# opensensor/thingino-accel

Measured on AMD Instinct MI355X. Metric: images/sec yolov5s_int8 640x640 batch256, higher is better.
Workload: dtype int8

## Files before the change

thingino-accel_amd/csrc/hip/conv_i8.hip:

```cpp
#include "conv_i8_common.hpp"

#ifndef I8M_ABL
#define I8M_ABL 0
#endif
template <int BPX, int BN, int STAGES, int KS = 1, int NW = 4>
__global__ __launch_bounds__(NW * 64) void conv_i8_mfma(const mhip_conv_i8_t p, const long total_pix, const int k64,
                                                         const int8_t *__restrict__ zeros, const unsigned noc,
                                                         const unsigned nblk, const int lg_inc, const unsigned kw_magic,
                                                         const fastdiv_t dhw, const fastdiv_t dow, const int bufmode,
                                                         const unsigned in_bytes) {
    ANAT_BEGIN();
    const bool POW2 = lg_inc >= 0;
    const bool masked = p.kh * p.kw <= 32;
    constexpr int SLICE = (BPX + BN) * BK;
    constexpr int STAGE = KS * SLICE;
    constexpr int NWN = BN == 128 ? 2 : 1;
    constexpr int NWM = NW / NWN;
    constexpr int WPX = BPX / NWM / 16;
    constexpr int WOC = BN / NWN / 16;
    constexpr int XROWS = BPX / NW;
    constexpr int XI = XROWS / 16;
    constexpr int LW = (BN / 16 + NW - 1) / NW;
    constexpr int L = XI + LW;
    static_assert(XI >= 1 && XROWS % 16 == 0, "every wave fetches whole 16-row pieces of the pixel tile");
// ... 1034 lines not shown

static int launch_variant(const mhip_conv_i8_t *p, long total_pix, int k64, const variant_t &v) {
    if (v.persist < 0) return -1;
    if (v.rows) return conv_i8_launch_rows(p);
    if (v.r128) return launch_r128(p, total_pix, v.r128);
    if (v.patch) return conv_i8_launch_patch(p, k64, v.patch);
    const int bn = p->oc_pad % 128 == 0 ? 128 : (p->oc_pad % 64 == 0 ? 64 : 32);
    const bool b16 = v.persist && v.stages == 2 && bn16_ok(p);
    if (v.bpx == 256) {
        if (bn == 128) return launch_variant_t<256, 128>(p, total_pix, k64, v);
        if (bn == 64) return launch_variant_t<256, 64>(p, total_pix, k64, v);
        if (b16) return launch_variant_t<256, 16>(p, total_pix, k64, v);
        return launch_variant_t<256, 32>(p, total_pix, k64, v);
    }
    if (bn == 128) return launch_variant_t<128, 128>(p, total_pix, k64, v);
    if (bn == 64) return launch_variant_t<128, 64>(p, total_pix, k64, v);
    if (b16) return launch_variant_t<128, 16>(p, total_pix, k64, v);
    return launch_variant_t<128, 32>(p, total_pix, k64, v);
}

template <int BPX, int BN>
static int launch_pair_t(const mhip_conv_i8_t *a, const mhip_conv_i8_t *b, long total_pix, int k64, int lg, unsigned magic,
                         int wres) {
    if (a->nseg > 1) return -2;
    return launch_persist_t<BPX, BN, 2, true, false, true>(a, total_pix, k64, lg, magic, b, wres);
}
extern "C" int mhip_conv_i8_pair(const mhip_conv_i8_t *a, const mhip_conv_i8_t *b) {
    if (!a || !b || !tune().persist || tune().variant) return -2;
    if (a->in != b->in || a->in_stride != b->in_stride || a->frames != b->frames || a->in_h != b->in_h || a->in_w != b->in_w ||
        a->in_c != b->in_c || a->out_h != b->out_h || a->out_w != b->out_w || a->kh != b->kh || a->kw != b->kw ||
        a->stride_h != b->stride_h || a->stride_w != b->stride_w || a->pad_top != b->pad_top || a->pad_left != b->pad_left ||
        a->row_pad != b->row_pad || a->nseg != b->nseg || a->seg_up != b->seg_up || !a->lut || !b->lut || a->add || b->add ||
        a->out_nchw || b->out_nchw)
        return -2;
    for (int i = 0; i < a->nseg; i++)
        if (a->seg_in[i] != b->seg_in[i] || a->seg_c[i] != b->seg_c[i] || a->seg_stride[i] != b->seg_stride[i]) return -2;
    if ((a->in_c % 16) != 0 || mhip_conv_i8_small_c(a->in_c, a->kw, a->out_c) || mhip_conv_i8_small_c(b->in_c, b->kw, b->out_c))
        return -2;
    if (a->nseg > 1 && (!seg_valid(a) || !seg_valid(b))) return -2;
    if (!persist_eligible(a) || !persist_eligible(b)) return -2;
    const int bn = a->oc_pad % 128 == 0 ? 128 : (a->oc_pad % 64 == 0 ? 64 : 32);
    const int bnb = b->oc_pad % 128 == 0 ? 128 : (b->oc_pad % 64 == 0 ? 64 : 32);
    if (bn != bnb || !mhip_zero_page()) return -2;
    const long total_pix = (long)a->frames * a->out_h * a->out_w;
    const int k64 = (a->kh * a->row_pad + BK - 1) / BK * BK, nks = k64 / BK;
    if (total_pix <= 0 || total_pix > 0x7fffffffL) return -2;
    int lg = 0;
    while ((1 << lg) < a->in_c) lg++;
    const unsigned magic = ((65536u + (unsigned)a->kw - 1u) / (unsigned)a->kw);
    const variant_t dv = default_variant(a, nks);
    const int bpx = dv.bpx ? dv.bpx : 128, wres = dv.persist && dv.wres && (tune().wres & 2);
    const bool b16 = bn16_ok(a) && bn16_ok(b);
    if (bpx == 256) {
        if (bn == 128) return launch_pair_t<256, 128>(a, b, total_pix, k64, lg, magic, wres);
        if (bn == 64) return launch_pair_t<256, 64>(a, b, total_pix, k64, lg, magic, wres);
        if (b16) return launch_pair_t<256, 16>(a, b, total_pix, k64, lg, magic, wres);
        return launch_pair_t<256, 32>(a, b, total_pix, k64, lg, magic, wres);
    }
    if (bn == 128) return launch_pair_t<128, 128>(a, b, total_pix, k64, lg, magic, wres);
    if (bn == 64) return launch_pair_t<128, 64>(a, b, total_pix, k64, lg, magic, wres);
    if (b16) return launch_pair_t<128, 16>(a, b, total_pix, k64, lg, magic, wres);
    return launch_pair_t<128, 32>(a, b, total_pix, k64, lg, magic, wres);
}

extern "C" int mhip_conv_i8_seg_ok(const mhip_conv_i8_t *p) {
    return p && (p->in_c % 16) == 0 && !mhip_conv_i8_small_c(p->in_c, p->kw, p->out_c) && seg_valid(p) && persist_eligible(p);
}

extern "C" int mhip_conv_i8_variants(const mhip_conv_i8_t *p, int *codes, int max) {
    if (!p || (p->in_c % 16) != 0 || mhip_conv_i8_small_c(p->in_c, p->kw, p->out_c)) return 0;
    const int k64 = (p->kh * p->row_pad + BK - 1) / BK * BK, nks = k64 / BK;
    int n = 0;
    if (p->pre_w) {
        const int first = conv_i8_pre_tile_rows(p);
        for (int th : {first, 16, 8, 4})
            if (th && n < max && conv_i8_patch_ok(p, th, nullptr)) {
                const int code = th == 16 ? 10 : (th == 8 ? 9 : 11);
                bool seen = false;
                for (int i = 0; i < n; i++) seen |= codes[i] == code;
                if (!seen) codes[n++] = code;
            }
        return n;
    }
    if (p->nseg > 1) {
        const int bn = p->oc_pad % 128 == 0 ? 128 : (p->oc_pad % 64 == 0 ? 64 : 32);
        const variant_t dv = default_variant(p, nks);
        const int dflt = dv.persist && dv.wres ? (dv.bpx == 256 ? 15 : 14) : (dv.bpx == 256 ? 4 : 2);
        if (n < max) codes[n++] = dflt;
        if (n < max && dflt != 2) codes[n++] = 2;
        if (n < max && dflt != 4) codes[n++] = 4;
        if (n < max && dflt != 14 && LUTB + 2 * (size_t)128 * BK + (size_t)nks * bn * BK <= 80 * 1024) codes[n++] = 14;
        if (n < max && dflt != 15 && LUTB + 2 * (size_t)256 * BK + (size_t)nks * bn * BK <= 80 * 1024) codes[n++] = 15;
        return n;
    }
    const int dflt = variant_code(default_variant(p, nks));
    if (n < max) codes[n++] = dflt;
    for (int code = 1; code <= NVARIANTS; code++) {
        const variant_t v = variant_of(code);
        if (code == dflt) continue;
        if (v.patch && !conv_i8_patch_ok(p, v.patch, nullptr)) continue;
        if (v.persist && !persist_eligible(p)) continue;
        if (v.ks2 && ((nks & 1) || nks < 4 || p->oc_pad % 64 != 0)) continue;
        if (v.w8 && (p->oc_pad % 128 != 0 || nks < 3)) continue;
        if (v.persist < 0) continue;
        if (v.r128 && !r128_ok(p)) continue;
        if (v.rows && !conv_i8_rows_ok(p)) continue;
        if (v.wres) {
            const int bn = p->oc_pad % 128 == 0 ? 128 : (p->oc_pad % 64 == 0 ? 64 : 32);
            if (LUTB + 2 * (size_t)v.bpx * BK + (size_t)nks * bn * BK > 80 * 1024) continue;
        }
        if (!v.persist && v.stages == 3 && nks <= 2) continue;
        if (n < max) codes[n++] = code;
    }
    return n;
}

template <int BN>
static int launch_generic(const mhip_conv_i8_t *p, long total_pix, int k64) {
    dim3 grid((unsigned)((total_pix + BP - 1) / BP), (unsigned)(p->oc_pad / BN));
    hipLaunchKernelGGL((conv_i8_generic<BN>), grid, dim3(NTHREADS), 0, mhip_stream_native(), *p, total_pix, k64,
                       make_fastdiv((unsigned)(p->out_h * p->out_w)));
    return mhip_check(hipGetLastError(), "conv_i8_generic launch");
}

extern "C" int mhip_conv_i8(const mhip_conv_i8_t *p) {
    if (!p || !p->in || !p->out || !p->w) return -1;
    if (p->out_pix_stride < 0 || p->out_ch_off < 0 || (p->out_nchw && (p->out_pix_stride || p->out_ch_off)) ||
        (p->out_pix_stride && p->out_pix_stride < p->out_ch_off + p->out_c))
        return -1;
    if (p->frames <= 0 || p->in_h <= 0 || p->in_w <= 0 || p->in_c <= 0 || p->out_h <= 0 || p->out_w <= 0 ||
        p->out_c <= 0 || p->kh <= 0 || p->kw <= 0 || p->stride_h < 0 || p->stride_w < 0)
        return -1;
    int row_pad, oc_pad;
    mhip_conv_i8_pack_geom(p->in_c, p->kw, p->out_c, &row_pad, &oc_pad, nullptr);
    if (row_pad != p->row_pad || oc_pad != p->oc_pad) return -1;
    if (p->add && (!p->safe || p->out_nchw || ((p->out_c | p->out_pix_stride | p->out_ch_off) & 15) || (p->in_c % 16) != 0 ||
                   mhip_conv_i8_small_c(p->in_c, p->kw, p->out_c) || p->nseg > 1))
        return -1;
    const long total_pix = (long)p->frames * p->out_h * p->out_w;
    const int k64 = (p->kh * p->row_pad + BK - 1) / BK * BK;
    if (total_pix <= 0 || total_pix > 0x7fffffffL || (total_pix + BP - 1) / BP * (oc_pad / 32) > 0x7fffffffL) return -1;
    if (p->in_planar) {
        if (p->in_planar > 4 || p->in_c != 4 || p->in_w < 4 || p->stride_h < 1 || p->stride_w < 1 || p->add || p->nseg > 1 ||
            !mhip_conv_i8_small_c(p->in_c, p->kw, p->out_c))
            return -2;
        return conv_i8_try_smallc(p, k64);
    }
    if (mhip_conv_i8_small_c(p->in_c, p->kw, p->out_c)) {
        if (p->stride_h >= 1 && p->stride_w >= 1) {
            int rc = conv_i8_try_rgb(p, k64);
            if (rc == -2) rc = conv_i8_try_smallc(p, k64);
            if (rc != -2) return rc;
        }
        if (p->add || p->nseg > 1) return -1;
        if (oc_pad % 64 == 0) return launch_generic<64>(p, total_pix, k64);
        return launch_generic<32>(p, total_pix, k64);
    }
    if (p->pre_w) {
        if (!mhip_zero_page() || !mhip_conv_i8_pre_ok(p)) return -1;
        int th = conv_i8_pre_tile_rows(p);
        const int code = p->variant ? p->variant : tune().variant;
        if (code >= 9 && code <= 11) {
            const int want = code == 10 ? 16 : (code == 9 ? 8 : 4);
            if (conv_i8_patch_ok(p, want, nullptr)) th = want;
        } else if (tune().small_batch && conv_i8_patch_ok(p, 4, nullptr) &&
                   ((long)p->frames * p->out_h * p->out_w + 255) / 256 * ((p->oc_pad + 127) / 128) < 256) {
            th = 4;
        }
        return conv_i8_launch_patch(p, k64, th);
    }
    if ((p->in_c % 16) == 0) {
        if (!mhip_zero_page()) return -1;
        const int nks = k64 / BK;
        if (p->variant < 0 || p->variant > NVARIANTS) return -1;
        int code = p->variant;
        if (p->nseg > 1) {
            if (!seg_valid(p) || !persist_eligible(p)) return -1;
            if (!code && tune().variant) {
                int codes[NVARIANTS];
                const int n = mhip_conv_i8_variants(p, codes, NVARIANTS);
                for (int i = 0; i < n; i++)
                    if (codes[i] == tune().variant) code = codes[i];
            }
            variant_t v = variant_of(code == 4 || code == 14 || code == 15 ? code : 2);
            if (!code) {
                const variant_t dv = default_variant(p, nks);
                v.bpx = dv.bpx ? dv.bpx : 128;
                v.wres = dv.persist && dv.wres;
            }
            return launch_variant(p, total_pix, k64, v);
        }
        if (!code && tune().variant) {
            int codes[NVARIANTS];
            const int n = mhip_conv_i8_variants(p, codes, NVARIANTS);
            for (int i = 0; i < n; i++)
                if (codes[i] == tune().variant) code = codes[i];
        }
        return launch_variant(p, total_pix, k64, code ? variant_of(code) : default_variant(p, nks));
    }
    if (oc_pad % 64 == 0) return launch_generic<64>(p, total_pix, k64);
    return launch_generic<32>(p, total_pix, k64);
}
```

thingino-accel_amd/csrc/hip/conv_i8_common.hpp:

```cpp
#pragma once
#include <hip/hip_runtime.h>
#include <stdint.h>
#include <stdlib.h>
#include <string.h>
#include <type_traits>

#include "../mhip.h"

extern "C" hipStream_t mhip_stream_native(void);
extern "C" int mhip_check(hipError_t e, const char *what);
extern "C" const void *mhip_zero_page(void);

typedef int v4i __attribute__((ext_vector_type(4)));
typedef int v2i __attribute__((ext_vector_type(2)));

#ifdef ANATOMY
struct anat_rec_t {
    unsigned key, wg, hwid, xcc;
    unsigned long long t[4];
};
static __device__ anat_rec_t *g_anat_buf;
static __device__ unsigned g_anat_cap;
#define ANAT_SETTER(NAME)                                                                                                    \
    extern "C" int NAME(void *buf, unsigned cap) {                                                                          \
// ... 318 lines not shown
                __builtin_memcpy(d, &v, 16);
            } else {
                const int rem = ncols - c * 16;
                int o = 0;
                if (rem & 8) { __builtin_memcpy(d, s, 8); o = 8; }
                if (rem & 4) { __builtin_memcpy(d + o, s + o, 4); o += 4; }
                if (rem & 2) { __builtin_memcpy(d + o, s + o, 2); o += 2; }
                if (rem & 1) d[o] = s[o];
            }
        }
    } else {
        for (int id = tid; id < BPX * BN; id += (int)blockDim.x) {
            const int c = id / BPX, row = id - c * BPX;
            const long off = rowoff[row];
            if (off < 0 || c >= ncols) continue;
            p.out[off + (size_t)(oc0 + c) * hw] = tile[row * ROW + c];
        }
    }
}

template <int BPX, int BN, int WPX, int WOC, bool LUT0 = false>
__device__ __forceinline__ void epilogue(const mhip_conv_i8_t &p, v4i (&acc)[WOC][WPX], int8_t *tile, const uint8_t *slut,
                                         const long *rowoff, int oc0, int pxw, int ocw, int hw) {
    const bool direct = !p.out_nchw && ((p.out_c | p.out_pix_stride | p.out_ch_off) & 15) == 0;
#define EPI(L, S, D) epilogue_t<BPX, BN, WPX, WOC, L, S, D, LUT0>(p, acc, tile, slut, rowoff, oc0, pxw, ocw, hw)
    if (direct) {
        if (p.lut) { if (p.safe) EPI(true, true, true); else EPI(true, false, true); }
        else { if (p.safe) EPI(false, true, true); else EPI(false, false, true); }
    } else {
        if (p.lut) { if (p.safe) EPI(true, true, false); else EPI(true, false, false); }
        else { if (p.safe) EPI(false, true, false); else EPI(false, false, false); }
    }
#undef EPI
}

template <int WPX, int WOC>
__device__ __forceinline__ void init_acc(const mhip_conv_i8_t &p, v4i (&acc)[WOC][WPX], int ocbase) {
    const int lane = threadIdx.x & 63;
#pragma unroll
    for (int s = 0; s < WOC; s++) {
        const v4i b = p.bias ? *(const v4i *)(p.bias + ocbase + s * 16 + (lane >> 4) * 4) : (v4i){0, 0, 0, 0};
#pragma unroll
        for (int t = 0; t < WPX; t++) acc[s][t] = b;
    }
}


struct tune_t {
    int init;
    int persist;
    int persist_stages;
    int persist_maxk;
    int persist_slots;
    int stages;
    int bpx;
    int variant;
    int bufmode;
    int small_batch;
    int rgb_direct;
    int wres;
    int few_wgs;
    int rows;
    int patch_ring;
    int patch_lds_kb;
};
const tune_t &conv_i8_tune_state();

extern "C" int mhip_conv_i8_small_c(int in_c, int kw, int out_c);

static inline long in_extent_bytes(const mhip_conv_i8_t *p) {
    return (long)(p->frames - 1) * (long)p->in_stride + (long)p->in_h * p->in_w * p->in_c;
}
static inline long persist_out_bytes(const mhip_conv_i8_t *p) {
    const long pstride = p->out_pix_stride ? p->out_pix_stride : p->out_c;
    return (long)(p->frames - 1) * (long)p->out_stride + (long)p->out_h * p->out_w * pstride;
}
static inline bool conv_i8_direct_rows(const mhip_conv_i8_t *p) {
    return !p->out_nchw && ((p->out_c | p->out_pix_stride | p->out_ch_off) & 15) == 0;
}

bool conv_i8_patch_ok(const mhip_conv_i8_t *p, int th, int *ring);
int conv_i8_launch_patch(const mhip_conv_i8_t *p, int k64, int th);
int conv_i8_pre_tile_rows(const mhip_conv_i8_t *p);
bool conv_i8_rows_ok(const mhip_conv_i8_t *p);
int conv_i8_launch_rows(const mhip_conv_i8_t *p);
int conv_i8_try_rgb(const mhip_conv_i8_t *p, int k64);
int conv_i8_try_smallc(const mhip_conv_i8_t *p, int k64);
```

thingino-accel_amd/csrc/hip/conv_i8_patch.hip:

```cpp
#include "conv_i8_common.hpp"
#include <stdio.h>

#ifdef PATCH_STAMPS
__device__ unsigned long long patch_stamp_sums[8];
extern "C" int mhip_patch_stamps(unsigned long long *out, int reset) {
    if (out && hipMemcpyFromSymbol(out, HIP_SYMBOL(patch_stamp_sums), sizeof(patch_stamp_sums)) != hipSuccess) return -1;
    if (reset) {
        unsigned long long z[8] = {0};
        if (hipMemcpyToSymbol(HIP_SYMBOL(patch_stamp_sums), z, sizeof(z)) != hipSuccess) return -1;
    }
    return 0;
}
#define STAMP(t)                                                                          \
    do {                                                                                  \
        __builtin_amdgcn_sched_barrier(0);                                                \
        asm volatile("s_memtime %0\n\ts_waitcnt lgkmcnt(0)" : "=s"(t)::"memory");        \
        __builtin_amdgcn_sched_barrier(0);                                                \
    } while (0)
#else
#define STAMP(t) do { } while (0)
#endif
#define PT_TW 16
#define PT_NIMAX 10

template <int LO, int HI>
__device__ __forceinline__ void wait_vmcnt_tree(int n) {
    if constexpr (LO == HI) {
        wait_vmcnt<LO>();
    } else {
        constexpr int MID = (LO + HI + 1) / 2;
        if (n >= MID) wait_vmcnt_tree<MID, HI>(n);
        else wait_vmcnt_tree<LO, MID - 1>(n);
    }
}
template <int HI>
__device__ __forceinline__ void wait_vmcnt_upto(int n) {
    wait_vmcnt_tree<0, HI>(n > HI ? HI : n);
}
__device__ __forceinline__ void barrier_lds() {
    asm volatile("s_waitcnt lgkmcnt(0)\n\ts_barrier" ::: "memory");
}

template <int TH, int BN, bool HAS_LUT, bool PRE = false>
__global__ __launch_bounds__(NTHREADS) void conv_i8_patch(const mhip_conv_i8_t p, const int k64, const int tiles_x,
                                                          const int tiles_y, const unsigned ntiles_all, const int PH,
                                                          const int PW, const int PWP, const int PWH, const int nblk,
                                                          const int8_t *__restrict__ zeros, const fastdiv_t dtx,
                                                          const fastdiv_t dty, const fastdiv_t dpwp, const unsigned out_bytes,
                                                          const int ring, const int xmap, const unsigned in_bytes) {
    ANAT_BEGIN();
    constexpr int WPX = TH / 4;
    constexpr int WOC = BN / 16;
    constexpr int NST = WPX;
    extern __shared__ __attribute__((aligned(16))) int8_t dynlds[];
    uint8_t *slut = (uint8_t *)dynlds;
    lds_base_must_be_zero(dynlds);
    const int nks = k64 / BK;
    constexpr int LB = LUTB + (PRE ? 512 : 0);
    int *dutab = (int *)(dynlds + LB);
    int8_t *wl = dynlds + LB + ((nks * 16 + 255) & ~255);
    const int patch_bytes = nblk * 1024;
    int8_t *w1l = wl + nks * BN * BK;
    int8_t *patch0 = w1l + (PRE ? p.in_c * BK : 0);
    int8_t *tpatch = patch0 + ring * patch_bytes;

    const int tid = threadIdx.x, lane = tid & 63;
    const int wv = __builtin_amdgcn_readfirstlane(tid >> 6);
    const int oc0 = blockIdx.y * BN;
    const int C = p.in_c, lgc = 31 - __builtin_clz((unsigned)C), cpp = C >> 4, lgcpp = lgc - 4;
    const int s = p.stride_w;
    const unsigned M = C >= 128 ? 6u : (C >= 64 ? 2u : 0u);

    v4i bias[WOC];
#pragma unroll
    for (int q = 0; q < WOC; q++) bias[q] = p.bias ? *(const v4i *)(p.bias + oc0 + q * 16 + (lane >> 4) * 4) : (v4i){0, 0, 0, 0};
    constexpr int W1MAX = 4;
    v4i pbias[PRE ? W1MAX : 1];
    if (PRE) {
#pragma unroll
        for (int q = 0; q < W1MAX; q++) pbias[q] = q < (C >> 4) ? *(const v4i *)(p.pre_bias + q * 16 + (lane >> 4) * 4) : (v4i){0, 0, 0, 0};
    }
    if (HAS_LUT) {
        if (p.lut2) { if (tid < 128) ((uint32_t *)slut)[tid] = ((const uint32_t *)p.lut2)[tid]; }
        else if (tid < 64) ((uint32_t *)slut)[tid] = ((const uint32_t *)p.lut)[tid];
    }
    if (PRE && tid >= 128) ((uint32_t *)slut)[tid] = ((const uint32_t *)p.pre_lut2)[tid - 128];
    const int rowbytes = p.kw * C, kbytes = p.kh * rowbytes;
    for (int i = tid; i < nks * 4; i += NTHREADS) {
        const int kb = i * 16;
        int du = 0;
        if (kb < kbytes) {
            const int ky = kb / rowbytes, rem = kb - ky * rowbytes, kx = rem >> lgc, cc = (rem & (C - 1)) >> 4;
            const int dp = ky * PWP + (s == 2 ? (kx >> 1) + (kx & 1) * PWH : kx);
            du = dp * cpp + cc;
        }
        dutab[i] = du;
    }
    __syncthreads();
    {
        const int schunk = (lane & 3) ^ (((lane >> 4) & 1) << 1);
        for (int i = wv; i < nks * (BN / 16); i += 4) {
            const int ks = i / (BN / 16), g = i - ks * (BN / 16);
            glds16(p.w + (size_t)(oc0 + g * 16 + (lane >> 2)) * k64 + ks * BK + schunk * 16, wl + (ks * BN + g * 16) * BK);
        }
        if (PRE)
            for (int g = wv; g < C / 16; g += 4) glds16(p.pre_w + (size_t)(g * 16 + (lane >> 2)) * BK + schunk * 16, w1l + g * 16 * BK);
    }
    int uoff[PT_NIMAX], upos[PT_NIMAX];
#pragma unroll
    for (int n = 0; n < PT_NIMAX; n++) {
        uoff[n] = 0;
        upos[n] = -1;
        if (n * 4 + wv < nblk) {
            const unsigned phys = (unsigned)((n * 4 + wv) * 64 + lane);
            const unsigned U = phys ^ ((phys >> 3) & M);
            const unsigned pp = U >> lgcpp, cc = U & (unsigned)(cpp - 1);
            const unsigned py = fdiv(pp, dpwp), col = pp - py * (unsigned)PWP;
            const int px = s == 2 ? ((int)col < PWH ? 2 * (int)col : 2 * ((int)col - PWH) + 1) : (int)col;
            if ((int)py < PH && px < PW) {
                uoff[n] = ((int)py * p.in_w + px) * C + (int)cc * 16;
                upos[n] = ((int)py << 16) | px;
            }
        }
    }
    const int npw = nblk > wv ? (nblk - wv + 3) >> 2 : 0;
    const unsigned xcd = blockIdx.x & 7u;
    const unsigned xstart = xmap ? (unsigned)(((unsigned long long)ntiles_all * xcd) >> 3) : 0u;
    const unsigned xend = xmap ? (unsigned)(((unsigned long long)ntiles_all * (xcd + 1u)) >> 3) : 0u;
    const unsigned ntiles = xmap ? (xend - xstart) * 8u + xcd : ntiles_all;
    auto tile_xy = [&](unsigned t, int &tx, int &ty, unsigned &f) {
        const unsigned j = xmap ? xstart + (t >> 3) : t, q = fdiv(j, dtx);
        tx = (int)(j - q * (unsigned)tiles_x);
        f = fdiv(q, dty);
        ty = (int)(q - f * (unsigned)tiles_y);
    };
    const __amdgpu_buffer_rsrc_t xrs = __builtin_amdgcn_make_buffer_rsrc((void *)p.in, 0, (int)in_bytes, 0x00020000);
    auto issue_patch = [&](unsigned t, int8_t *dst) {
#ifdef PATCH_ABL
        return;
#endif
        int tx, ty;
        unsigned f;
        tile_xy(t, tx, ty, f);
        const int iy0 = ty * TH * s - p.pad_top, ix0 = tx * PT_TW * s - p.pad_left;
        if (in_bytes != 0u && iy0 >= 0 && ix0 >= 0 && iy0 + PH <= p.in_h && ix0 + PW <= p.in_w) {
            const int sbase = (int)(f * (unsigned)p.in_stride) + (iy0 * p.in_w + ix0) * C;
#pragma unroll
            for (int n = 0; n < PT_NIMAX; n++)
                if (n * 4 + wv < nblk) blds16(xrs, uoff[n], sbase, dst + (n * 4 + wv) * 1024);
            return;
        }
        const int8_t *base = p.in + (size_t)f * p.in_stride + ((long)iy0 * p.in_w + ix0) * C;
#pragma unroll
        for (int n = 0; n < PT_NIMAX; n++)
            if (n * 4 + wv < nblk) {
                const int py = upos[n] >> 16, px = upos[n] & 0xffff;
                const bool ok = upos[n] >= 0 && (unsigned)(iy0 + py) < (unsigned)p.in_h && (unsigned)(ix0 + px) < (unsigned)p.in_w;
                glds16(ok ? base + uoff[n] : zeros, dst + (n * 4 + wv) * 1024);
            }
    };

    const __amdgpu_buffer_rsrc_t orsrc = __builtin_amdgcn_make_buffer_rsrc(p.out, 0, (int)out_bytes, 0x00020000);
    const bool has_add = p.add != nullptr;
    constexpr int RROW = WOC == 4 ? 1024 : 512;
    constexpr int NRI = WOC == 4 ? WPX : 2 * WPX;
    int8_t *rstage = patch0 + (ring + (PRE ? 1 : 0)) * patch_bytes + wv * (WPX * RROW);
    const int NR = has_add ? NRI : 0;
    const int frow = lane & 15, fchunk = lane >> 4;
    const int chan = (lane >> 4) * (4 * WOC);
    const int pstride = p.out_pix_stride ? p.out_pix_stride : p.out_c;
    const int lo = p.relu ? 0 : -128;
    const uint8_t *lut128 = slut + 128;
    int ubase[WPX];
#pragma unroll
    for (int u = 0; u < WPX; u++) ubase[u] = ((wv * WPX + u) * s * PWP + frow) * cpp;

    const unsigned G = gridDim.x;
    const int D = ring - 1;
    unsigned t = blockIdx.x;
    int yg0 = 0, yg1 = 0, yg2 = 0;
    {
        int issued = 0;
        for (int d = 0; d < D; d++)
            if (t + (unsigned)d * G < ntiles) {
                issue_patch(t + (unsigned)d * G, patch0 + d * patch_bytes);
                issued++;
            }
        yg0 = issued > 1 ? (issued - 1) * npw : 0;
        yg1 = issued > 2 ? (issued - 2) * npw : 0;
        yg2 = 0;
    }
#ifdef PATCH_STAMPS
    unsigned long long st0 = 0, st1 = 0, st2 = 0, st3 = 0, st4 = 0, sum_wait = 0, sum_issue = 0, sum_k = 0, sum_epi = 0, sum_tiles = 0;
#endif
    int cur = 0;
    int pn_last = 0;
    bool first = true;
    ANAT_NOW(1);
    for (; t < ntiles; t += G) {
        STAMP(st0);
        int tx, ty;
        unsigned f;
        tile_xy(t, tx, ty, f);
        int voffs[WPX];
        uint32_t xw[WPX][WOC];
#pragma unroll
        for (int u = 0; u < WPX; u++) {
            const int oy = ty * TH + wv * WPX + u, ox = tx * PT_TW + frow;
            const unsigned off = f * (unsigned)p.out_stride + (unsigned)(oy * p.out_w + ox) * (unsigned)pstride +
                                 (unsigned)(p.out_ch_off + oc0 + chan);
            const bool ok = oy < p.out_h && ox < p.out_w && oc0 + chan < p.out_c;
            voffs[u] = ok ? (int)off : -1;
#pragma unroll
            for (int q = 0; q < WOC; q++) xw[u][q] = 0;
        }
        if (has_add) {
#pragma unroll
            for (int u = 0; u < WPX; u++) {
                const int8_t *src = voffs[u] >= 0 ? p.add + (unsigned)voffs[u] : zeros;
                if (WOC == 4) {
                    glds16(src, rstage + u * RROW);
                } else {
                    __builtin_amdgcn_global_load_lds((const __attribute__((address_space(1))) void *)src,
                                                     (__attribute__((address_space(3))) void *)(rstage + u * RROW), 4, 0, 0);
                    __builtin_amdgcn_global_load_lds((const __attribute__((address_space(1))) void *)(src + 4),
                                                     (__attribute__((address_space(3))) void *)(rstage + u * RROW + 256), 4, 0, 0);
                }
            }
        }
        if (D > 0) {
            wait_vmcnt_upto<63>(yg0 + NR);
            barrier_lds();
            STAMP(st1);
            const unsigned tn = t + (unsigned)D * G;
            int pn = 0;
            if (tn < ntiles) {
                int slot = cur + D;
                slot = slot >= ring ? slot - ring : slot;
                issue_patch(tn, patch0 + slot * patch_bytes);
                pn = npw;
            }
            const int after = NR + pn + NST;
            yg0 = yg1 + after;
            yg1 = yg2 + after;
            yg2 = NST;
            if (D == 1) yg0 = NST;
            if (D == 2) yg1 = NST;
            pn_last = pn;
        } else {
            if (!first) barrier_lds();
            issue_patch(t, patch0);
            wait_vmcnt<0>();
            barrier_lds();
        }
        first = false;
        STAMP(st2);
        const int8_t *patch = patch0 + cur * patch_bytes;
        if (PRE) {
            const int WOC1 = C >> 4;
            const int P = PH * PWP, nsub = (P + 15) >> 4;
            const int iy0 = ty * TH * s - p.pad_top, ix0 = tx * PT_TW * s - p.pad_left;
            for (int sub = wv; sub < nsub; sub += 4) {
                int pp = sub * 16 + frow;
                const bool live = pp < P;
                pp = live ? pp : P - 1;
                const unsigned Ur = (unsigned)(pp * cpp + (fchunk & (cpp - 1)));
                const v4i xb1 = *(const v4i *)(patch + ((Ur ^ ((Ur >> 3) & M)) << 4));
                const unsigned py = fdiv((unsigned)pp, dpwp), px = (unsigned)pp - py * (unsigned)PWP;
                const bool inimg = live && (int)py < PH && (int)px < PW && (unsigned)(iy0 + (int)py) < (unsigned)p.in_h &&
                                   (unsigned)(ix0 + (int)px) < (unsigned)p.in_w;
                uint32_t pk1[W1MAX];
                if (WOC1 == 4) {
                    int a1[16];
#pragma unroll
                    for (int q = 0; q < 4; q++) {
                        const v4i wa = *(const v4i *)(w1l + lds_off(q * 16 + frow, fchunk));
                        const v4i r = __builtin_amdgcn_mfma_i32_16x16x64_i8(wa, xb1, pbias[PRE ? q : 0], 0, 0, 0);
#pragma unroll
                        for (int e = 0; e < 4; e++) a1[q * 4 + e] = r[e];
                    }
                    uint32_t pk4[4];
                    requant_pack_pre<16>(a1, p.pre_cs, pk4);
#pragma unroll
                    for (int e = 0; e < 4; e++) pk1[e] = inimg ? pk4[e] : 0u;
                    const unsigned Uw = (unsigned)(pp * cpp + (lane >> 4));
                    if (live) *(v4i *)(tpatch + ((Uw ^ ((Uw >> 3) & M)) << 4)) = (v4i){(int)pk1[0], (int)pk1[1], (int)pk1[2], (int)pk1[3]};
                } else {
                    int a1[8];
#pragma unroll
                    for (int q = 0; q < 2; q++) {
                        const v4i wa = *(const v4i *)(w1l + lds_off(q * 16 + frow, fchunk));
                        const v4i r = __builtin_amdgcn_mfma_i32_16x16x64_i8(wa, xb1, pbias[PRE ? q : 0], 0, 0, 0);
#pragma unroll
                        for (int e = 0; e < 4; e++) a1[q * 4 + e] = r[e];
                    }
                    uint32_t pk2[2];
                    requant_pack_pre<8>(a1, p.pre_cs, pk2);
                    const int g4 = lane >> 4;
                    const unsigned Uw = (unsigned)(pp * cpp + (g4 >> 1));
                    if (live)
                        *(uint2 *)(tpatch + ((Uw ^ ((Uw >> 3) & M)) << 4) + (g4 & 1) * 8) = make_uint2(inimg ? pk2[0] : 0u, inimg ? pk2[1] : 0u);
                }
            }
            barrier_lds();
            patch = tpatch;
        }
        v4i acc[WOC][WPX];
        v4i xa[WPX], wa[WOC], xb[WPX], wb[WOC];
        auto load_frags = [&](int ks, int du, v4i (&xf)[WPX], v4i (&wf)[WOC]) {
#pragma unroll
            for (int u = 0; u < WPX; u++) {
                const unsigned U = (unsigned)(ubase[u] + du);
                xf[u] = *(const v4i *)(patch + ((U ^ ((U >> 3) & M)) << 4));
            }
            const int8_t *ws = wl + ks * BN * BK;
#pragma unroll
            for (int q = 0; q < WOC; q++) wf[q] = *(const v4i *)(ws + lds_off(q * 16 + frow, fchunk));
        };
        auto mfma_step = [&](const v4i (&xf)[WPX], const v4i (&wf)[WOC]) {
#pragma unroll
            for (int q = 0; q < WOC; q++)
#pragma unroll
                for (int u = 0; u < WPX; u++) acc[q][u] = __builtin_amdgcn_mfma_i32_16x16x64_i8(wf[q], xf[u], acc[q][u], 0, 0, 0);
        };
        const int last = nks - 1;
        auto clampk = [&](int k) { return k < last ? k : last; };
        load_frags(0, dutab[fchunk], xa, wa);
        load_frags(clampk(1), dutab[clampk(1) * 4 + fchunk], xb, wb);
        int du_n = dutab[clampk(2) * 4 + fchunk];
#pragma unroll
        for (int q = 0; q < WOC; q++)
#pragma unroll
            for (int u = 0; u < WPX; u++) acc[q][u] = __builtin_amdgcn_mfma_i32_16x16x64_i8(wa[q], xa[u], bias[q], 0, 0, 0);
        int ks = 1;
        for (; ks + 1 < nks; ks += 2) {
            load_frags(ks + 1, du_n, xa, wa);
            du_n = dutab[clampk(ks + 2) * 4 + fchunk];
            __builtin_amdgcn_sched_barrier(0);
            mfma_step(xb, wb);
            __builtin_amdgcn_sched_barrier(0);
            load_frags(clampk(ks + 2), du_n, xb, wb);
            du_n = dutab[clampk(ks + 3) * 4 + fchunk];
            __builtin_amdgcn_sched_barrier(0);
            mfma_step(xa, wa);
            __builtin_amdgcn_sched_barrier(0);
        }
        if (ks < nks) mfma_step(xb, wb);
        STAMP(st3);
        if (D > 0) cur = cur + 1 == ring ? 0 : cur + 1;
        if (has_add) {
            if (D > 0) wait_vmcnt_upto<15>(pn_last);
#pragma unroll
            for (int u = 0; u < WPX; u++) {
                if (WOC == 4) {
                    const v4i r = *(const v4i *)(rstage + u * RROW + lane * 16);
                    xw[u][0] = (uint32_t)r[0]; xw[u][1] = (uint32_t)r[1]; xw[u][WOC > 2 ? 2 : 0] = (uint32_t)r[2]; xw[u][WOC > 3 ? 3 : 0] = (uint32_t)r[3];
                } else {
                    xw[u][0] = *(const uint32_t *)(rstage + u * RROW + lane * 4);
                    xw[u][WOC > 1 ? 1 : 0] = *(const uint32_t *)(rstage + u * RROW + 256 + lane * 4);
                }
            }
        }
#pragma unroll
        for (int u = 0; u < WPX; u++) {
            uint32_t pk[WOC];
            int a[WOC * 4];
#pragma unroll
            for (int q = 0; q < WOC; q++)
#pragma unroll
                for (int r = 0; r < 4; r++) a[q * 4 + r] = acc[q][u][r];
            const bool fast = HAS_LUT && p.lut2 != nullptr;
            if (has_add) {
                const add_args_t ga = {p.add_s_conv, p.add_s_other, p.add_inv};
                if (fast) requant_pack<WOC * 4, HAS_LUT, true, true, true, true>(a, p.cs, lo, lut128, pk, xw[u], &ga);
                else requant_pack<WOC * 4, HAS_LUT, true, true, true>(a, p.cs, lo, lut128, pk, xw[u], &ga);
            } else {
                if (fast) requant_pack<WOC * 4, HAS_LUT, true, true, false, true>(a, p.cs, lo, lut128, pk);
                else requant_pack<WOC * 4, HAS_LUT, true, true>(a, p.cs, lo, lut128, pk);
            }
            const int voff = voffs[u];
            if (WOC == 4)
                __builtin_amdgcn_raw_buffer_store_b128((v4i){(int)pk[0], (int)pk[1], (int)pk[2], (int)pk[3]}, orsrc, voff, 0, 0);
            else if (WOC == 2)
                __builtin_amdgcn_raw_buffer_store_b64((v2i){(int)pk[0], (int)pk[WOC > 1 ? 1 : 0]}, orsrc, voff, 0, 0);
        }
#ifdef PATCH_STAMPS
        STAMP(st4);
        if (D == 0) st1 = st2;
        sum_wait += st1 - st0; sum_issue += st2 - st1; sum_k += st3 - st2; sum_epi += st4 - st3; sum_tiles += 1;
#endif
    }
    ANAT_NOW(2);
    ANAT_END(p);
#ifdef PATCH_STAMPS
    if (lane == 0) {
        atomicAdd(&patch_stamp_sums[0], sum_wait); atomicAdd(&patch_stamp_sums[1], sum_issue); atomicAdd(&patch_stamp_sums[2], sum_k);
        atomicAdd(&patch_stamp_sums[3], sum_epi); atomicAdd(&patch_stamp_sums[4], sum_tiles);
    }
#endif
}

ANAT_SETTER(mhip_anatomy_set_patch)
struct patch_geom_t {
    int bn, tiles_x, tiles_y, PH, PW, PWP, PWH, nblk, nks, ring;
    size_t lds;
};
static inline const tune_t &tune() { return conv_i8_tune_state(); }
static size_t patch_lds_budget(int bn) {
    const int kb = tune().patch_lds_kb;
    if (kb >= 16 && kb <= 160 && kb != 80) return (size_t)kb * 1024;
    return (size_t)(bn == 32 ? 53 : 80) * 1024;
}
static bool patch_geom(const mhip_conv_i8_t *p, int th, patch_geom_t *g) {
    const bool direct = conv_i8_direct_rows(p);
    const int C = p->in_c, s = p->stride_w;
    static const bool no_c16 = getenv("MARS_HIP_PATCH_NO_C16") != nullptr;
    if (!direct || !p->safe || (C != 16 && C != 32 && C != 64 && C != 128) || (C == 16 && (no_c16 || p->pre_w)) || (s != 1 && s != 2) || p->stride_h != s ||
        p->kh > 7 || p->kw > 7 || p->kh * p->kw < 2 || p->row_pad != p->kw * C || persist_out_bytes(p) > 0x7fffffffL)
        return false;
    const int k64 = (p->kh * p->row_pad + BK - 1) / BK * BK;
    g->nks = k64 / BK;
    g->bn = p->oc_pad % 64 == 0 ? 64 : 32;
    g->tiles_x = (p->out_w + PT_TW - 1) / PT_TW;
    g->tiles_y = (p->out_h + th - 1) / th;
    if ((double)p->out_h * p->out_w < (C == 128 ? 0.80 : 0.85) * (double)g->tiles_x * PT_TW * g->tiles_y * th) return false;
    g->PH = (th - 1) * s + p->kh;
    g->PW = (PT_TW - 1) * s + p->kw;
    g->PWH = s == 2 ? (g->PW + 1) / 2 : 0;
    g->PWP = s == 2 ? 2 * g->PWH : g->PW;
    const long units = (long)g->PH * g->PWP * (C / 16);
    g->nblk = (int)((units + 63) / 64);
    if (g->nblk > 4 * PT_NIMAX) return false;
    const bool pre = p->pre_w != nullptr;
    if (pre && (s != 1 || (C != 32 && C != 64) || !p->pre_bias || !p->pre_lut2 || !p->lut2)) return false;
    const size_t pb = (size_t)g->nblk * 1024;
    const size_t radd = p->add ? (size_t)4 * (th / 4) * (g->bn == 64 ? 1024 : 512) : 0;
    const size_t fixed = LUTB + (pre ? 512 + (size_t)C * BK + pb : 0) + (((size_t)g->nks * 16 + 255) & ~(size_t)255) +
                         (size_t)g->nks * g->bn * BK + radd;
    const size_t budget = patch_lds_budget(g->bn);
    if (fixed + pb > budget) return false;
    const int fit = (int)((budget - fixed) / pb);
    const int cap = tune().patch_ring > 0 ? (tune().patch_ring > 4 ? 4 : tune().patch_ring) : 2;
    int ring = fit < cap ? fit : cap;
    g->ring = ring;
    g->lds = fixed + (size_t)ring * pb;
    if ((long)g->tiles_x * g->tiles_y * p->frames > 0x7fffffffL) return false;
    return true;
}

template <int TH, int BN, bool HAS_LUT, bool PRE = false>
static int launch_patch_t(const mhip_conv_i8_t *p, int k64, const patch_geom_t &g) {
    auto kern = conv_i8_patch<TH, BN, HAS_LUT, PRE>;
    static int cus = 0;
    static size_t slots_lds[8];
    static int slots_n[8], nslots = 0;
    if (!cus) {
        int dev = 0;
        hipDeviceProp_t prop;
        if (hipFuncSetAttribute((const void *)kern, hipFuncAttributeMaxDynamicSharedMemorySize, 160 * 1024) != hipSuccess ||
            hipGetDevice(&dev) != hipSuccess || hipGetDeviceProperties(&prop, dev) != hipSuccess)
            return mhip_check(hipErrorUnknown, "conv_i8_patch occupancy query");
        cus = prop.multiProcessorCount;
    }
    int slots = 0;
    for (int i = 0; i < nslots; i++)
        if (slots_lds[i] == g.lds) slots = slots_n[i];
    if (!slots) {
        int occ = 0;
        if (hipOccupancyMaxActiveBlocksPerMultiprocessor(&occ, kern, NTHREADS, g.lds) != hipSuccess)
            return mhip_check(hipErrorUnknown, "conv_i8_patch occupancy query");
        slots = (occ > 0 ? occ : 1) * cus;
        if (nslots < 8) { slots_lds[nslots] = g.lds; slots_n[nslots++] = slots; }
    }
    const unsigned ntiles = (unsigned)((long)g.tiles_x * g.tiles_y * p->frames);
    const unsigned noc = (unsigned)(p->oc_pad / BN);
    unsigned gx = (unsigned)(tune().persist_slots > 0 ? tune().persist_slots : slots) / noc;
    if (gx < 1) gx = 1;
    if (gx > ntiles) gx = ntiles;
    const int xmap = gx >= 8 && ntiles < 0x0fffffffu;
    if (xmap) gx &= ~7u;
    {
        static const char *dbg = getenv("MARS_HIP_PATCH_DEBUG");
        static size_t last_lds = 0;
        static int last_ring = 0;
        if (dbg && (last_lds != g.lds || last_ring != g.ring)) {
            fprintf(stderr, "Mars: conv_i8_patch<%d,%d> ring %d, patch %d KB, LDS %zu B, %d workgroups per CU, grid %u x %u\n", TH, BN, g.ring,
                    g.nblk, g.lds, slots / cus, gx, noc);
            last_lds = g.lds;
            last_ring = g.ring;
        }
    }
    hipLaunchKernelGGL(kern, dim3(gx, noc), dim3(NTHREADS), g.lds, mhip_stream_native(), *p, k64,
                       g.tiles_x, g.tiles_y, ntiles, g.PH, g.PW, g.PWP, g.PWH, g.nblk, (const int8_t *)mhip_zero_page(),
                       make_fastdiv((unsigned)g.tiles_x), make_fastdiv((unsigned)g.tiles_y), make_fastdiv((unsigned)g.PWP),
                       (unsigned)persist_out_bytes(p), g.ring, xmap,
                       in_extent_bytes(p) <= 0x7fffffffL ? (unsigned)in_extent_bytes(p) : 0u);
    return mhip_check(hipGetLastError(), "conv_i8_patch launch");
}

bool conv_i8_patch_ok(const mhip_conv_i8_t *p, int th, int *ring) {
    patch_geom_t g;
    if (!patch_geom(p, th, &g)) return false;
    if (ring) *ring = g.ring;
    return true;
}

int conv_i8_launch_patch(const mhip_conv_i8_t *p, int k64, int th) {
    patch_geom_t g;
    if (!patch_geom(p, th, &g)) return -1;
#define PATCH(T, B)                                                                       \
    (p->pre_w ? launch_patch_t<T, B, true, true>(p, k64, g)                               \
              : (p->lut ? launch_patch_t<T, B, true>(p, k64, g) : launch_patch_t<T, B, false>(p, k64, g)))
    if (th == 16) return g.bn == 64 ? PATCH(16, 64) : PATCH(16, 32);
    if (th == 8) return g.bn == 64 ? PATCH(8, 64) : PATCH(8, 32);
    return g.bn == 64 ? PATCH(4, 64) : PATCH(4, 32);
#undef PATCH
}

int conv_i8_pre_tile_rows(const mhip_conv_i8_t *p) {
    patch_geom_t g;
    for (int th : {16, 8, 4})
        if (patch_geom(p, th, &g) && (th == 4 || g.ring >= 2)) return th;
    return 0;
}
extern "C" int mhip_conv_i8_pre_ok(const mhip_conv_i8_t *p) {
    if (!p || !p->pre_w || p->nseg > 1 || p->out_nchw) return 0;
    return conv_i8_pre_tile_rows(p) != 0;
}
```

thingino-accel_amd/csrc/host/mars_internal.h:

```cpp
#ifndef MARS_INTERNAL_H
#define MARS_INTERNAL_H

#include <stddef.h>
#include <stdint.h>

#include "../mhip.h"
#include "mars_hip.h"
#include "mars_runtime.h"

enum {
    OP_CONV_I8 = 0,
    OP_CONV_F32,
    OP_RELU_BYTES,
    OP_LUT_I8,
    OP_BINARY_I8,
    OP_SIGMOID_F32,
    OP_BINARY_F32,
    OP_RELU_F32,
    OP_BN,
    OP_MAXPOOL,
    OP_CONCAT_SLICE,
    OP_UPSAMPLE,
    OP_UPSAMPLE_Q, OP_MAXPOOL_Q,
    OP_CONCAT_Q,
    OP_CONV_F32_VHEAD,
    OP_FAIL,
};

#define NO_OFF ((size_t)-1)
#define MARS_MAX_IO 4
#define MARS_MAX_MODEL_TUNE 16

typedef struct {
    size_t bytes;
    size_t extent;
    size_t stride;
    uint8_t *dev;
    int is_weight;
    int needed;
    int io_in, io_out;
    uint8_t *host;
    uint8_t *dense_dev;
    int pix_c, pix_stride;
    int rec_c, rec_hw;
    int nhwc_c, nhwc_hw;
    size_t zero_from;
    int partial;
    int nhwc_pitch;
    int tail_read;
} mtensor_t;

typedef struct {
    int kind, layer, err;
    int t_in[4], n_in, t_out;
    int in_h, in_w, in_c, out_h, out_w, out_c, kh, kw, sh, sw, pt, pl;
    int nchw, relu, is_mul, is_f32, leaky, safe;
    size_t in_byte_off, out_byte_off;
    int k_limit;
    int vc_n, vc_t[3], vc_run, vc_shift;
    int rows_only;
    int out_nchw;
    int silu_f32;
    int f32_exact;
    int variant;
    int add_t; float add_s_conv, add_s_other, add_inv;
    int nseg, seg_t[4], seg_c[4], seg_up;
    int chain_n, chain_out[3];
    int pair_next;
    int row_pad, oc_pad, c_pad;
    int ch_off, scale_h, scale_w, bn_n;
    int out_pix_stride, out_ch_off;
    int store_c;
    float cs, f0, f1, f2;
    size_t n;
    size_t w_off, b_off, lut_off, s_off;
    int pre;
    size_t pre_w_off, pre_b_off, pre_lut2_off;
    float pre_cs;
    size_t w2_off;
    int w2_rows;
    int w2_planes;
    size_t w3_off;
    int w3_stem;
    int in_rec, out_rec;
    size_t lut2_off;
    size_t w_blob_off[2];
    double macs, bytes;
    int prof_kind;
    float last_ms;
    void *ev0, *ev1;
    int prof_rec;
    void *ev_start;
} mars_op_t;

typedef struct {
    int fusion;
    unsigned no_fuse_lut : 1, no_nhwc_internal : 1, no_vconcat_q : 1, no_pair_f32 : 1, no_rec : 1, no_zero_tail : 1, no_vconcat_f32 : 1,
        no_rowpad : 1;
    size_t rec_limit;
    size_t vconcat_limit;
    size_t bottleneck_limit;
} plan_switches_t;

typedef struct mars_model_ext {
    mars_model_t pub;
    plan_switches_t sw;
    int batch, profiling, deferred;
    int plan_err;
    int no_vconcat;
    int no_download;
    int no_bottleneck;
    int rec_frames;
    int rec_skipped;
    size_t rec_max_frames;
    mtensor_t *mt;
    mars_op_t *ops;
    int n_ops, cap_ops;
    uint8_t *arena_host;
    size_t arena_size, arena_cap;
    uint8_t *arena_dev;
    size_t blob_mirror_bytes;
    uint8_t *act_dev;
    size_t act_bytes;
    uint8_t *scratch_dev;
    size_t scratch_per_frame;
    int scratch_t, scratch_cpad, scratch_f0, scratch_n;
    void *det_dev;
    int *det_counts_dev;
    float *det_lut_dev;
    int det_cap;
    float det_lut_scale[4];
    int det_lut_n;
    int det_lut_mono[4];
    float *heads_lut_dev;
    float heads_lut_scale[4];
    int heads_lut_n;
    float *dfl_lut_dev;
    float dfl_lut_scale[4][2];
    int dfl_lut_n;
    void *ev_graph_done, *ev_tail_done;
    int tail_pending;
    int frame0, run_frames;
    void *ev_fork, *ev_join[3];
    void *ev_chunk[2][8];
    void *graph_exec;
    unsigned graph_gen;
    int ran_plain;
    void *pipe;
    struct { char key[28]; int value, saved; } tune[MARS_MAX_MODEL_TUNE];
    int n_tune, tune_depth;
    int plan_f32_mode;
    unsigned char *layer_noop;
    void *roi_dev;
    int roi_cap_slots, roi_cap_frames;
    int roi_slots;
    struct mars_model_ext *roi_from;
    void *cls_dev;
    size_t cls_bytes, cls_sums_off, cls_top_off;
    int cls_frames, cls_c, cls_top_k;
    void *ev_label_done;
    int label_pending;
    void *label_dev;
    int label_cap, label_frames;
    void *match_dev;
    size_t match_bytes, match_top_off, match_row_off;
    int match_frames, match_top_k;
    void *ident_dev;
    int ident_cap, ident_frames;
    void *track_dev;
    int track_cap, track_frames;
    void *seg_dev;
    size_t seg_bytes, seg_rec_off, seg_word_off;
    int seg_frames, seg_max, seg_ph, seg_pw;
    void *ev_seg[2];
    void *pose_dev;
    size_t pose_bytes, pose_rec_off, pose_kpt_off;
    int pose_frames, pose_max, pose_k;
    float pose_lut_scale[4];
    int pose_lut_n;
    void *ev_pose[2];
    struct mars_model_ext *live_next;
} mars_model_ext_t;


#define MARS_INTERNAL __attribute__((visibility("hidden")))
#define ALIGN_UP(x, a) (((x) + (size_t)(a) - 1) & ~((size_t)(a) - 1))
#define NO_TENSOR 0xFFFFFFFFu
#define MAX_DIM_PRODUCT ((size_t)1 << 40)
#define ARENA_MAX ((size_t)1 << 40)
#define MAX_CHANNELS 65536
MARS_INTERNAL int mars_verbose(void);
#define VLOG(...) do { if (mars_verbose()) fprintf(stderr, "Mars: " __VA_ARGS__); } while (0)
MARS_INTERNAL void drop_graph(mars_model_ext_t *m);
MARS_INTERNAL mars_model_ext_t *mars_live_models(void);
MARS_INTERNAL void plan_switches_read(plan_switches_t *sw, int at_load);
MARS_INTERNAL mars_error_t build_plan(mars_model_ext_t *m);
MARS_INTERNAL mars_error_t upload_params(mars_model_ext_t *m);
MARS_INTERNAL mars_error_t alloc_batch(mars_model_ext_t *m, int n);
MARS_INTERNAL size_t elem_size(uint32_t dtype);
MARS_INTERNAL size_t shape_numel(const mars_tensor_t *d);
MARS_INTERNAL size_t reference_buffer_size(const mars_model_ext_t *m);
MARS_INTERNAL size_t arena_reserve(mars_model_ext_t *m, size_t bytes);
MARS_INTERNAL void blob_read(const mars_model_ext_t *m, size_t off, size_t n, void *dst);
MARS_INTERNAL int op_reads(const mars_op_t *o, int t);
MARS_INTERNAL int op_writes(const mars_op_t *o, int t);
MARS_INTERNAL size_t planned_stride(const mtensor_t *t);
MARS_INTERNAL void conv_i8_geometry(const mars_op_t *op, int frames, mhip_conv_i8_t *p);
MARS_INTERNAL int conv_i8_pre_fits(const mars_op_t *op, int frames, size_t in_stride, size_t out_stride);
MARS_INTERNAL void plan_layer(mars_model_ext_t *m, int li);
MARS_INTERNAL void fold_silu(mars_model_ext_t *m, int f32);
MARS_INTERNAL void fuse_lut(mars_model_ext_t *m);
MARS_INTERNAL void nhwc_internal(mars_model_ext_t *m);
MARS_INTERNAL void fold_add(mars_model_ext_t *m, int f32);
MARS_INTERNAL void virtual_concat(mars_model_ext_t *m);
MARS_INTERNAL void elide_concat(mars_model_ext_t *m);
MARS_INTERNAL void trim_concat(mars_model_ext_t *m);
MARS_INTERNAL void fuse_pool_chains(mars_model_ext_t *m);
MARS_INTERNAL void pair_convs(mars_model_ext_t *m);
MARS_INTERNAL void fuse_bottleneck(mars_model_ext_t *m);
MARS_INTERNAL void pad_output_rows(mars_model_ext_t *m);
MARS_INTERNAL void virtual_concat_q(mars_model_ext_t *m);
MARS_INTERNAL void f32_policy(mars_model_ext_t *m);
MARS_INTERNAL void zero_tail_f32(mars_model_ext_t *m);
MARS_INTERNAL void pair_convs_f32(mars_model_ext_t *m);
MARS_INTERNAL void rec_pairs(mars_model_ext_t *m);
MARS_INTERNAL void virtual_concat_f32(mars_model_ext_t *m);
MARS_INTERNAL void plan_check(mars_model_ext_t *m);
MARS_INTERNAL void conv_i8_params(const mars_model_ext_t *m, const mars_op_t *op, mhip_conv_i8_t *p);
MARS_INTERNAL int mars_preproc_prepare(int w, int h, int tw, int th);
MARS_INTERNAL int mars_preproc_prepare_nv12(int w, int h, int tw, int th, int frames);

MARS_INTERNAL void mars_roi_release(mars_model_ext_t *m);

MARS_INTERNAL void mars_cls_release(mars_model_ext_t *m);

MARS_INTERNAL void mars_match_release(mars_model_ext_t *m);

MARS_INTERNAL void mars_track_release(mars_model_ext_t *m);

MARS_INTERNAL void mars_seg_release(mars_model_ext_t *m);

MARS_INTERNAL void mars_pose_release(mars_model_ext_t *m);

MARS_INTERNAL int mars_tensor_chw(const mars_tensor_t *d, int *c, int *h, int *w);
MARS_INTERNAL int mars_locate_i8(const mars_model_ext_t *m, int T, int ch, int hh, int ww, int any_writer, int *buf, int *off, int *pix_step, int *ch_step);
MARS_INTERNAL mars_error_t mars_own_det_buffers(mars_model_ext_t *m);
MARS_INTERNAL mars_error_t mars_tail_on_aux(mars_model_ext_t *m, int (*launch)(struct mars_model_ext *, const void *, void *, int *), const void *cfg);

mars_error_t mars_detect_prepare(mars_model_ext_t *m, const int *output_indices, int n_outputs);
int mars_detect_launch(mars_model_ext_t *m, const int *output_indices, int n_outputs, float nms_thresh, void *dets_dev,
                       int *counts_dev);

typedef struct {
    int n, ti[4], stride[4], nc[4], h[4], w[4], pix_step[4], ch_step[4];
    float anchors[4][3][2];
    float conf, nms;
    int map, px, py;
    float rx, ry;
    int internal;
} mars_heads_cfg_t;
MARS_INTERNAL int mars_find_heads(const mars_model_ext_t *m, int *tensor_ids, int *strides, int *num_classes, int cap);
MARS_INTERNAL mars_error_t mars_heads_resolve(mars_model_ext_t *m, const mars_yolo_heads_t *h, mars_heads_cfg_t *c);
MARS_INTERNAL mars_error_t mars_heads_prepare(mars_model_ext_t *m, const mars_heads_cfg_t *c);
MARS_INTERNAL int mars_heads_launch(mars_model_ext_t *m, const mars_heads_cfg_t *c, void *dets_dev, int *counts_dev);

typedef struct {
    int n, reg_max, stride[4], nc[4], h[4], w[4];
    int box_t[4], cls_t[4], box_buf[4], cls_buf[4], box_off[4], cls_off[4];
    int box_pix_step[4], box_ch_step[4], cls_pix_step[4], cls_ch_step[4];
    float box_scale[4], cls_scale[4];
    float conf, nms;
    int map, px, py;
    float rx, ry;
    int internal;
    int *cand_pred, *kept_pred;
    void *premap;
} mars_dfl_cfg_t;
MARS_INTERNAL int mars_find_dfl_heads(const mars_model_ext_t *m, int *box_ids, int *cls_ids, int *strides, int *num_classes, int *reg_max, int cap);
MARS_INTERNAL mars_error_t mars_dfl_resolve(mars_model_ext_t *m, const mars_yolo_dfl_heads_t *h, mars_dfl_cfg_t *c);
MARS_INTERNAL mars_error_t mars_dfl_prepare(mars_model_ext_t *m, const mars_dfl_cfg_t *c);
MARS_INTERNAL int mars_dfl_launch(mars_model_ext_t *m, const mars_dfl_cfg_t *c, void *dets_dev, int *counts_dev);

int32_t mars_trunc_x86(float x);
void mars_pack_conv_i8(const int8_t *w, size_t avail, int nchw, int out_c, int in_c, int kh, int kw,
                       int c_pad, int row_pad, int oc_pad, int8_t *dst);

#endif
```

thingino-accel_amd/csrc/host/mars_model.c:

```c
#include <math.h>
#include <stdio.h>
#include <stdlib.h>
#include <string.h>
#include <sys/types.h>
#include <time.h>

#include "mars_internal.h"
#include "nna.h"


int mars_verbose(void) {
    static int v = -1;
    if (v < 0) v = getenv("MARS_VERBOSE") ? 1 : 0;
    return v;
}

void plan_switches_read(plan_switches_t *sw, int at_load) {
    const char *e;
    if (at_load) sw->fusion = (e = getenv("MARS_HIP_FUSION")) ? atoi(e) : 1;
    sw->no_fuse_lut = getenv("MARS_HIP_NO_FUSE_LUT") != NULL;
    sw->no_nhwc_internal = getenv("MARS_HIP_NO_NHWC_INTERNAL") != NULL;
    sw->no_vconcat_q = getenv("MARS_HIP_NO_VCONCAT_Q") != NULL;
    sw->no_pair_f32 = getenv("MARS_HIP_NO_PAIR_F32") != NULL;
    sw->no_rec = getenv("MARS_HIP_NO_REC") != NULL;
    sw->no_zero_tail = getenv("MARS_HIP_NO_ZERO_TAIL") != NULL;
    sw->no_vconcat_f32 = getenv("MARS_HIP_NO_VCONCAT_F32") != NULL;
    sw->no_rowpad = getenv("MARS_HIP_NO_ROWPAD") != NULL;
    sw->rec_limit = (e = getenv("MARS_HIP_REC_LIMIT")) ? (size_t)strtoull(e, NULL, 0) : (size_t)0xfffffff0u;
    sw->vconcat_limit = (e = getenv("MARS_HIP_VCONCAT_LIMIT")) ? (size_t)strtoull(e, NULL, 0) : (size_t)0x7fffffffu;
    sw->bottleneck_limit = (e = getenv("MARS_HIP_BOTTLENECK_LIMIT")) ? (size_t)strtoull(e, NULL, 0) : 0;
}

void drop_graph(mars_model_ext_t *m) {
    if (m->graph_exec) {
        mhip_sync();
        mhip_graph_destroy(m->graph_exec);
    }
    m->graph_exec = NULL;
    m->ran_plain = 0;
}

static const char *const k_err[] = {
    "OK", "Invalid magic number", "Version mismatch", "Memory allocation failed",
    "Invalid file format", "NNA initialization failed", "Layer execution failed",
    "Invalid tensor", "Invalid layer",
};

const char *mars_get_error_string(mars_error_t err) {
    int i = -(int)err;
    if (i >= 0 && i < (int)(sizeof(k_err) / sizeof(k_err[0]))) return k_err[i];
    return "Unknown error";
}

static void free_device_state(mars_model_ext_t *m) {
    drop_graph(m);
    if (m->act_dev) mhip_free(m->act_dev);
    if (m->scratch_dev) mhip_free(m->scratch_dev);
    m->act_dev = m->scratch_dev = NULL;
    for (uint32_t i = 0; m->mt && i < m->pub.header.num_tensors; i++) {
        if (m->mt[i].host) mhip_host_free(m->mt[i].host);
        m->mt[i].host = NULL;
        if (m->mt[i].dense_dev) mhip_free(m->mt[i].dense_dev);
        m->mt[i].dense_dev = NULL;
        if (!m->mt[i].is_weight) m->mt[i].dev = NULL;
    }
    if (m->det_dev) mhip_free(m->det_dev);
    if (m->det_counts_dev) mhip_free(m->det_counts_dev);
    m->det_dev = NULL;
    m->det_counts_dev = NULL;
    m->det_cap = 0;
    m->tail_pending = 0;
    mars_roi_release(m);
    mars_cls_release(m);
    mars_track_release(m);
    mars_seg_release(m);
    mars_pose_release(m);
}

static void free_ops(mars_model_ext_t *m) {
    drop_graph(m);
    for (int i = 0; i < m->n_ops; i++) {
        if (m->ops[i].ev0) mhip_event_destroy(m->ops[i].ev0);
        if (m->ops[i].ev1) mhip_event_destroy(m->ops[i].ev1);
    }
    free(m->ops);
    m->ops = NULL;
    m->n_ops = m->cap_ops = 0;
}

static mars_model_ext_t *g_live_models = NULL;
mars_model_ext_t *mars_live_models(void) { return g_live_models; }

void mars_free(mars_model_t *model) {
    if (!model) return;
    mars_model_ext_t *m = (mars_model_ext_t *)model;
    for (mars_model_ext_t **pp = &g_live_models; *pp; pp = &(*pp)->live_next)
        if (*pp == m) { *pp = m->live_next; break; }
    for (mars_model_ext_t *x = g_live_models; x; x = x->live_next)
        if (x->roi_from == m) x->roi_from = NULL;
    if (m->pipe) mars_hip_pipe_close(model);
    if (mhip_ready()) mhip_sync();
    free_device_state(m);
    free_ops(m);
    if (m->arena_dev) mhip_free(m->arena_dev);
    if (m->det_lut_dev) mhip_free(m->det_lut_dev);
    if (m->heads_lut_dev) mhip_free(m->heads_lut_dev);
    if (m->dfl_lut_dev) mhip_free(m->dfl_lut_dev);
    if (m->ev_graph_done) mhip_event_destroy(m->ev_graph_done);
    if (m->ev_tail_done) mhip_event_destroy(m->ev_tail_done);
    if (m->ev_label_done) mhip_event_destroy(m->ev_label_done);
    if (m->ev_fork) mhip_event_destroy(m->ev_fork);
    for (int k = 0; k < 3; k++)
        if (m->ev_join[k]) mhip_event_destroy(m->ev_join[k]);
    for (int k = 0; k < 2; k++)
        for (int c = 0; c < 8; c++)
            if (m->ev_chunk[k][c]) mhip_event_destroy(m->ev_chunk[k][c]);
    free(m->arena_host);
    free(m->layer_noop);
    free(m->mt);
    free(m->pub.weights);
    free(m->pub.layers);
    free(m->pub.tensors);
    free(m);
}

mars_error_t build_plan(mars_model_ext_t *m) {
    const uint32_t nt = m->pub.header.num_tensors, nl = m->pub.header.num_layers;
    plan_switches_read(&m->sw, 0);
    free_ops(m);
    m->arena_size = 0;
    if (m->arena_host) memset(m->arena_host, 0, m->arena_cap);
    m->scratch_per_frame = 0;
    m->plan_err = MARS_OK;
    m->plan_f32_mode = mhip_conv_f32_mode(-1);
    m->blob_mirror_bytes = m->pub.weights_size;
    for (uint32_t i = 0; i < nt; i++) {
        m->mt[i].extent = m->mt[i].bytes;
        m->mt[i].pix_c = m->mt[i].pix_stride = 0;
        m->mt[i].needed = (m->mt[i].io_in || m->mt[i].io_out) ? 1 : 0;
    }
    for (uint32_t i = 0; i < nl && m->plan_err == MARS_OK; i++) {
        const int n0 = m->n_ops;
        plan_layer(m, (int)i);
        m->layer_noop[i] = m->n_ops == n0;
    }
    if (m->plan_err != MARS_OK) return (mars_error_t)m->plan_err;
    if (m->sw.fusion >= 1) {
        fold_silu(m, 0);
        fuse_lut(m);
        fold_silu(m, 1);
        nhwc_internal(m);
        fold_add(m, 0);
        fold_add(m, 1);
        if (!m->no_vconcat) virtual_concat(m);
        elide_concat(m);
        trim_concat(m);
        fuse_pool_chains(m);
        pair_convs(m);
        if (m->sw.fusion >= 2 && !m->no_bottleneck) fuse_bottleneck(m);
        pad_output_rows(m);
        virtual_concat_q(m);
    } else {
        nhwc_internal(m);
    }
    f32_policy(m);
    zero_tail_f32(m);
    if (m->sw.fusion >= 1) pair_convs_f32(m);
    rec_pairs(m);
    virtual_concat_f32(m);
    if (m->plan_err == MARS_OK) plan_check(m);
    return (mars_error_t)m->plan_err;
}

mars_error_t upload_params(mars_model_ext_t *m) {
    size_t mirror_off = arena_reserve(m, m->blob_mirror_bytes + 64);
    if (mirror_off == NO_OFF) return MARS_ERR_ALLOC_FAILED;
    if (!m->deferred) blob_read(m, 0, m->blob_mirror_bytes, m->arena_host + mirror_off);
    if (m->arena_dev) mhip_free(m->arena_dev);
    m->arena_dev = (uint8_t *)mhip_malloc(m->arena_size);
    if (!m->arena_dev) return MARS_ERR_ALLOC_FAILED;
    if (mhip_h2d_async(m->arena_dev, m->arena_host, m->arena_size) || mhip_sync()) return MARS_ERR_NNA_INIT_FAILED;
    for (uint32_t i = 0; i < m->pub.header.num_tensors; i++) {
        if (!m->mt[i].is_weight) continue;
        m->mt[i].dev = m->arena_dev + mirror_off + (size_t)m->pub.tensors[i].desc.data_offset;
        m->mt[i].stride = 0;
        m->pub.tensors[i].paddr = m->mt[i].dev;
    }
    m->pub.ddr_paddr = m->arena_dev;
    m->pub.ddr_size = m->arena_size;
    return MARS_OK;
}

mars_error_t alloc_batch(mars_model_ext_t *m, int n) {
    const uint32_t nt = m->pub.header.num_tensors;
    if (m->pipe) mars_hip_pipe_close(&m->pub);
    if (mhip_sync()) return MARS_ERR_LAYER_FAILED;
    plan_switches_read(&m->sw, 0);
    const size_t vlim = m->sw.vconcat_limit, blim = m->sw.bottleneck_limit;
    const int rec_replan = (size_t)n > m->rec_max_frames || (m->rec_skipped && n < m->rec_frames);
    m->rec_frames = n;
    if (m->no_vconcat || m->no_bottleneck || rec_replan) {
        m->no_vconcat = m->no_bottleneck = 0;
        mars_error_t e = build_plan(m);
        if (e == MARS_OK) e = upload_params(m);
        if (e != MARS_OK) return e;
    }
    if (!m->no_vconcat)
        for (int i = 0; i < m->n_ops; i++) {
            const mars_op_t *op = &m->ops[i];
            if (op->kind != OP_CONV_I8 || op->nseg < 2 || op->t_out < 0) continue;
            if (planned_stride(&m->mt[op->t_out]) * (size_t)n > vlim) {
                m->no_vconcat = 1;
                mars_error_t e = build_plan(m);
                if (e == MARS_OK) e = upload_params(m);
                if (e != MARS_OK) return e;
                break;
            }
        }
    if (m->sw.fusion >= 2 && !m->no_bottleneck)
        for (int i = 0; i < m->n_ops; i++) {
            const mars_op_t *op = &m->ops[i];
            if (op->kind != OP_CONV_I8 || !op->pre || op->t_out < 0) continue;
            const size_t in_stride = op->t_in[0] >= 0 ? planned_stride(&m->mt[op->t_in[0]]) : 0;
            if (!conv_i8_pre_fits(op, n, in_stride, planned_stride(&m->mt[op->t_out])) || (blim && (size_t)n > blim)) {
                m->no_bottleneck = 1;
                mars_error_t e = build_plan(m);
                if (e == MARS_OK) e = upload_params(m);
                if (e != MARS_OK) return e;
                break;
            }
        }
    free_device_state(m);
    size_t per_frame = 0;
    for (uint32_t i = 0; i < nt; i++) {
        mtensor_t *t = &m->mt[i];
        if (t->is_weight || !t->needed) continue;
        t->stride = planned_stride(t);
        per_frame += t->stride;
    }
    m->act_bytes = per_frame * (size_t)n;
    m->act_dev = (uint8_t *)mhip_malloc(m->act_bytes + 512);
    if (!m->act_dev) return MARS_ERR_ALLOC_FAILED;
    if (mhip_memset_async(m->act_dev, 0, m->act_bytes + 256)) return MARS_ERR_ALLOC_FAILED;
    size_t off = 256;
    for (uint32_t i = 0; i < nt; i++) {
        mtensor_t *t = &m->mt[i];
        mars_runtime_tensor_t *rt = &m->pub.tensors[i];
        if (t->is_weight) continue;
        rt->vaddr = NULL; rt->paddr = NULL; rt->alloc_size = 0;
        if (!t->needed) continue;
        t->dev = m->act_dev + off;
        off += t->stride * (size_t)n;
        rt->paddr = t->dev;
        rt->alloc_size = t->stride * (size_t)n;
        if (t->io_in || t->io_out) {
            const size_t hb = t->bytes * (size_t)n, ref = reference_buffer_size(m);
            size_t cap = hb > ref ? hb : ref;
            if (ref > ((size_t)8 << 20)) cap = hb;
            t->host = (uint8_t *)mhip_host_alloc(cap ? cap : 64);
            if (!t->host) return MARS_ERR_ALLOC_FAILED;
            memset(t->host, 0, cap);
            rt->vaddr = t->host;
            rt->alloc_size = n == 1 && cap >= ref ? ref : hb;
        }
        if (t->pix_stride) {
            t->dense_dev = (uint8_t *)mhip_malloc(t->bytes * (size_t)n);
            if (!t->dense_dev) return MARS_ERR_ALLOC_FAILED;
        }
    }
    if (m->scratch_per_frame) {
        m->scratch_dev = (uint8_t *)mhip_malloc(ALIGN_UP(m->scratch_per_frame, 256) * (size_t)n + 256);
        if (!m->scratch_dev) return MARS_ERR_ALLOC_FAILED;
    }
    m->batch = n;
    m->frame0 = 0;
    m->run_frames = n;
    return mhip_sync() ? MARS_ERR_ALLOC_FAILED : MARS_OK;
}

static mars_error_t load_host(const void *data, size_t size, unsigned flags, mars_model_ext_t **out_m) {
    if (!data || !out_m || size < sizeof(mars_header_t)) return MARS_ERR_INVALID_FILE;
    const uint8_t *p = (const uint8_t *)data;
    mars_header_t h;
    memcpy(&h, p, sizeof(h));
    if (h.magic != MARS_MAGIC) {
        VLOG("Invalid magic 0x%08x (expected 0x%08x)\n", h.magic, MARS_MAGIC);
        return MARS_ERR_INVALID_MAGIC;
    }
    if (h.version_major != MARS_VERSION_MAJOR) return MARS_ERR_VERSION_MISMATCH;
    if (h.num_tensors > 65536 || h.num_layers > 65536 || h.num_inputs > 4 || h.num_outputs > 4) return MARS_ERR_INVALID_FILE;
    const size_t tables = sizeof(h) + (size_t)h.num_tensors * sizeof(mars_tensor_t) + (size_t)h.num_layers * sizeof(mars_layer_t);
    if (tables > size) return MARS_ERR_INVALID_FILE;
    const int deferred = (flags & MARS_HIP_LOAD_DEFER_WEIGHTS) != 0;
    if (!deferred && h.weights_size > 0 && (h.weights_offset > size || h.weights_size > size - h.weights_offset))
        return MARS_ERR_INVALID_FILE;
    if (h.weights_size > ((uint64_t)1 << 36)) return MARS_ERR_INVALID_FILE;

    mars_model_ext_t *m = (mars_model_ext_t *)calloc(1, sizeof(*m));
    if (!m) return MARS_ERR_ALLOC_FAILED;
    m->pub.header = h;
    plan_switches_read(&m->sw, 1);
    m->deferred = deferred;
    m->pub.tensors = (mars_runtime_tensor_t *)calloc(h.num_tensors ? h.num_tensors : 1, sizeof(mars_runtime_tensor_t));
    m->pub.layers = (mars_runtime_layer_t *)calloc(h.num_layers ? h.num_layers : 1, sizeof(mars_runtime_layer_t));
    m->mt = (mtensor_t *)calloc(h.num_tensors ? h.num_tensors : 1, sizeof(mtensor_t));
    m->layer_noop = (unsigned char *)calloc(h.num_layers ? h.num_layers : 1, 1);
    if (!m->pub.tensors || !m->pub.layers || !m->mt || !m->layer_noop) { mars_free(&m->pub); return MARS_ERR_ALLOC_FAILED; }
    const uint8_t *q = p + sizeof(h);
    for (uint32_t i = 0; i < h.num_tensors; i++, q += sizeof(mars_tensor_t)) memcpy(&m->pub.tensors[i].desc, q, sizeof(mars_tensor_t));
    for (uint32_t i = 0; i < h.num_layers; i++, q += sizeof(mars_layer_t)) memcpy(&m->pub.layers[i].desc, q, sizeof(mars_layer_t));

    m->pub.weights_size = (size_t)h.weights_size;
    if (h.weights_size) {
        m->pub.weights = calloc(1, (size_t)h.weights_size);
        if (!m->pub.weights) { mars_free(&m->pub); return MARS_ERR_ALLOC_FAILED; }
        if (!deferred) memcpy(m->pub.weights, p + h.weights_offset, (size_t)h.weights_size);
    }
    m->pub.ddr_base = m->pub.weights;
    for (uint32_t i = 0; i < h.num_tensors; i++) {
        mars_runtime_tensor_t *rt = &m->pub.tensors[i];
        if (rt->desc.ndims > MARS_MAX_DIMS) { mars_free(&m->pub); return MARS_ERR_INVALID_FILE; }
        m->mt[i].bytes = shape_numel(&rt->desc) * elem_size(rt->desc.dtype);
        if (rt->desc.data_size > 0) {
            if (rt->desc.data_offset > h.weights_size) { mars_free(&m->pub); return MARS_ERR_INVALID_FILE; }
            m->mt[i].is_weight = 1;
            rt->vaddr = (uint8_t *)m->pub.weights + rt->desc.data_offset;
            rt->alloc_size = (size_t)rt->desc.data_size;
        }
    }
    for (uint32_t i = 0; i < h.num_inputs; i++) {
        uint32_t id = h.input_tensor_ids[i];
        if (id < h.num_tensors && !m->mt[id].is_weight) m->mt[id].io_in = (int)i + 1;
    }
    for (uint32_t i = 0; i < h.num_outputs; i++) {
        uint32_t id = h.output_tensor_ids[i];
        if (id < h.num_tensors && !m->mt[id].is_weight) m->mt[id].io_out = (int)i + 1;
    }

    mars_error_t err = build_plan(m);
    if (err != MARS_OK) { mars_free(&m->pub); return err; }
    VLOG("%u layers -> %d launches, parameter arena %zu bytes\n", h.num_layers, m->n_ops, m->arena_size);
    *out_m = m;
    return MARS_OK;
}

mars_error_t mars_hip_load_memory_ex(const void *data, size_t size, unsigned flags, mars_model_t **out_model) {
    if (!out_model) return MARS_ERR_INVALID_FILE;
    mars_model_ext_t *m = NULL;
    mars_error_t err = load_host(data, size, flags, &m);
    if (err != MARS_OK) return err;
    if (!nna_is_ready() || !mhip_ready()) {
        fprintf(stderr, "Mars: no initialised MI355X device (call nna_init first); refusing to load\n");
        mars_free(&m->pub);
        return MARS_ERR_NNA_INIT_FAILED;
    }
    err = upload_params(m);
    if (err == MARS_OK) err = alloc_batch(m, 1);
    if (err != MARS_OK) { mars_free(&m->pub); return err; }
    m->live_next = g_live_models;
    g_live_models = m;
    *out_model = &m->pub;
    return MARS_OK;
}

static int describe_op_full(const mars_op_t *o, char *line, size_t cap, int k) {
#define ADD(...) k += snprintf(line + k, cap - (size_t)k, __VA_ARGS__)
    ADD(" | err %d in %dx%dx%d out %dx%dx%d k %dx%d s %dx%d p %d,%d", o->err, o->in_h, o->in_w, o->in_c, o->out_h, o->out_w, o->out_c, o->kh, o->kw, o->sh, o->sw, o->pt, o->pl);
    ADD(" nchw %d out_nchw %d relu %d is_mul %d is_f32 %d leaky %d safe %d silu %d f32_exact %d variant %d", o->nchw, o->out_nchw, o->relu, o->is_mul, o->is_f32, o->leaky,
        o->safe, o->silu_f32, o->f32_exact, o->variant);
    ADD(" row_pad %d oc_pad %d c_pad %d store_c %d ch_off %d out_ch_off %d out_pix_stride %d in_byte_off %zu out_byte_off %zu scale %dx%d bn_n %d n %zu", o->row_pad,
        o->oc_pad, o->c_pad, o->store_c, o->ch_off, o->out_ch_off, o->out_pix_stride, o->in_byte_off, o->out_byte_off, o->scale_h, o->scale_w, o->bn_n, o->n);
    ADD(" k_limit %d rows_only %d pair_next %d in_rec %d out_rec %d vc %d,%d,%d:", o->k_limit, o->rows_only, o->pair_next, o->in_rec, o->out_rec, o->vc_n, o->vc_run, o->vc_shift);
    for (int q = 0; q < o->vc_n && q < 3; q++) ADD(" %d", o->vc_t[q]);
    ADD(" add %d %a %a %a seg %d up %d:", o->add_t, (double)o->add_s_conv, (double)o->add_s_other, (double)o->add_inv, o->nseg, o->seg_up);
    for (int q = 0; q < o->nseg && q < 4; q++) ADD(" %d/%d", o->seg_t[q], o->seg_c[q]);
    ADD(" chain %d:", o->chain_n);
    for (int q = 0; q < o->chain_n && q < 3; q++) ADD(" %d", o->chain_out[q]);
    ADD(" cs %a f %a %a %a", (double)o->cs, (double)o->f0, (double)o->f1, (double)o->f2);
    ADD(" w_off %zd b_off %zd lut_off %zd lut2_off %zd s_off %zd w2_off %zd rows %d planes %d w3_off %zd stem %d blob %zd %zd", (ssize_t)o->w_off, (ssize_t)o->b_off,
        (ssize_t)o->lut_off, (ssize_t)o->lut2_off, (ssize_t)o->s_off, (ssize_t)o->w2_off, o->w2_rows, o->w2_planes, (ssize_t)o->w3_off, o->w3_stem, (ssize_t)o->w_blob_off[0],
        (ssize_t)o->w_blob_off[1]);
    ADD(" pre %d", o->pre);
    if (o->pre) ADD(" %zd %zd %zd %a", (ssize_t)o->pre_w_off, (ssize_t)o->pre_b_off, (ssize_t)o->pre_lut2_off, (double)o->pre_cs);
    ADD(" macs %a bytes %a prof_kind %d", o->macs, o->bytes, o->prof_kind);
#undef ADD
    return k;
}

size_t mars_hip_describe_plan(const void *data, size_t size, unsigned flags, char *out, size_t cap) {
    static const char *const kinds[] = {"conv_i8", "conv_f32", "relu_bytes", "lut_i8", "binary_i8", "sigmoid_f32", "binary_f32", "relu_f32", "bn",
                                        "maxpool", "concat_slice", "upsample", "upsample_q", "maxpool_q", "concat_q", "conv_f32_vhead", "fail"};
    mars_model_ext_t *m = NULL;
    const int full = (flags & MARS_HIP_DESCRIBE_FULL) != 0;
    if (load_host(data, size, flags & ~MARS_HIP_DESCRIBE_FULL, &m) != MARS_OK) return 0;
    size_t n = 0;
    char line[4096];
#define EMIT() do { const size_t l = strlen(line); if (out && n < cap) memcpy(out + n, line, n + l <= cap ? l : cap - n); n += l; } while (0)
    for (int i = 0; i < m->n_ops; i++) {
        const mars_op_t *o = &m->ops[i];
        int k = snprintf(line, sizeof line, "op %d layer %d %s in", i, o->layer, o->kind >= 0 && o->kind <= OP_FAIL ? kinds[o->kind] : "?");
        for (int q = 0; q < o->n_in && q < 4; q++) k += snprintf(line + k, sizeof line - (size_t)k, " %d", o->t_in[q]);
        k += snprintf(line + k, sizeof line - (size_t)k, " out %d", o->t_out);
#define FLAG(cond, ...) if (cond) k += snprintf(line + k, sizeof line - (size_t)k, __VA_ARGS__)
        FLAG(o->kind == OP_CONV_I8 || o->kind == OP_CONV_F32 || o->kind == OP_CONV_F32_VHEAD, " k%dx%d s%d c%d->%d", o->kh, o->kw, o->sw, o->in_c, o->out_c);
        FLAG(o->nchw, " relayout"); FLAG(o->out_nchw, " planar_store"); FLAG(o->lut_off != NO_OFF, " lut"); FLAG(o->add_t, " add=%d", o->add_t - 1);
        FLAG(o->nseg, " seg=%d", o->nseg); FLAG(o->pair_next, " pair_next"); FLAG(o->pre, " pre"); FLAG(o->silu_f32, " silu");
        FLAG(o->k_limit, " k_limit=%d", o->k_limit); FLAG(o->in_rec, " in_rec=%d", o->in_rec); FLAG(o->out_rec, " out_rec");
        FLAG(o->vc_shift, " view=-%d", o->vc_shift); FLAG(o->vc_n, " vcat=%dx%d", o->vc_n, o->vc_run);
        FLAG(o->rows_only, " rows_only=%d", o->rows_only); FLAG(o->out_byte_off, " out_off=%zu", o->out_byte_off); FLAG(o->chain_n, " chain=%d", o->chain_n);
        FLAG(o->out_pix_stride, " pix_stride=%d", o->out_pix_stride); FLAG(o->kind == OP_FAIL, " err=%d", o->err);
#undef FLAG
        if (full) k = describe_op_full(o, line, sizeof line, k);
        snprintf(line + k, sizeof line - (size_t)k, "\n");
        EMIT();
    }
    for (uint32_t t = 0; t < m->pub.header.num_tensors; t++) {
        const mtensor_t *mt = &m->mt[t];
        const int listed = mt->nhwc_c || mt->partial || mt->zero_from || mt->rec_c || mt->pix_stride;
        if (!listed && !(full && mt->needed)) continue;
        int k = listed ? snprintf(line, sizeof line, "tensor %u nhwc_c %d pitch %d partial %d zero_from %zu rec_c %d pix_stride %d", t, mt->nhwc_c, mt->nhwc_pitch,
                                  mt->partial, mt->zero_from, mt->rec_c, mt->pix_stride)
                       : snprintf(line, sizeof line, "+tensor %u", t);
        if (full)
            k += snprintf(line + k, sizeof line - (size_t)k, " | bytes %zu extent %zu needed %d tail_read %d weight %d io %d,%d pix_c %d rec_hw %d nhwc_hw %d", mt->bytes,
                          mt->extent, mt->needed, mt->tail_read, mt->is_weight, mt->io_in, mt->io_out, mt->pix_c, mt->rec_hw, mt->nhwc_hw);
        snprintf(line + k, sizeof line - (size_t)k, "\n");
        EMIT();
    }
    if (full) {
        const plan_switches_t *w = &m->sw;
        snprintf(line, sizeof line, "+plan n_ops %d arena_size %zu scratch_per_frame %zu blob_mirror_bytes %zu rec_max_frames %zu rec_skipped %d f32_mode %d | fusion %d"
                 " no_fuse_lut %d no_nhwc_internal %d no_vconcat_q %d no_pair_f32 %d no_rec %d no_zero_tail %d no_vconcat_f32 %d no_rowpad %d rec_limit %zu"
                 " vconcat_limit %zu bottleneck_limit %zu\n", m->n_ops, m->arena_size, m->scratch_per_frame, m->blob_mirror_bytes, m->rec_max_frames, m->rec_skipped,
                 m->plan_f32_mode, w->fusion, w->no_fuse_lut, w->no_nhwc_internal, w->no_vconcat_q, w->no_pair_f32, w->no_rec, w->no_zero_tail, w->no_vconcat_f32,
                 w->no_rowpad, w->rec_limit, w->vconcat_limit, w->bottleneck_limit);
        EMIT();
    }
#undef EMIT
    if (out && cap) out[n < cap ? n : cap - 1] = 0;
    mars_free(&m->pub);
    return n;
}

int mars_yolo_find_heads(const void *data, size_t size, int *tensor_ids, int *strides, int *num_classes, int cap) {
    mars_model_ext_t *m = NULL;
    if (load_host(data, size, 0, &m) != MARS_OK) return -1;
    const int n = mars_find_heads(m, tensor_ids, strides, num_classes, cap);
    mars_free(&m->pub);
    return n;
}

int mars_yolo_find_dfl_heads(const void *data, size_t size, int *box_ids, int *cls_ids, int *strides, int *num_classes, int *reg_max, int cap) {
    mars_model_ext_t *m = NULL;
    if (load_host(data, size, 0, &m) != MARS_OK) return -1;
    const int n = mars_find_dfl_heads(m, box_ids, cls_ids, strides, num_classes, reg_max, cap);
    mars_free(&m->pub);
    return n;
}

mars_error_t mars_load_memory(const void *data, size_t size, mars_model_t **model) {
    return mars_hip_load_memory_ex(data, size, 0, model);
}

mars_error_t mars_load_file(const char *path, mars_model_t **model) {
    if (!path || !model) return MARS_ERR_INVALID_FILE;
    FILE *fp = fopen(path, "rb");
    if (!fp) {
        fprintf(stderr, "Mars: Cannot open %s\n", path);
        return MARS_ERR_INVALID_FILE;
    }
    fseek(fp, 0, SEEK_END);
    long size = ftell(fp);
    fseek(fp, 0, SEEK_SET);
    if (size <= 0) { fclose(fp); return MARS_ERR_INVALID_FILE; }
    void *buf = malloc((size_t)size);
    if (!buf) { fclose(fp); return MARS_ERR_ALLOC_FAILED; }
    if (fread(buf, 1, (size_t)size, fp) != (size_t)size) { free(buf); fclose(fp); return MARS_ERR_INVALID_FILE; }
    fclose(fp);
    mars_error_t err = mars_load_memory(buf, (size_t)size, model);
    free(buf);
    return err;
}

mars_runtime_tensor_t *mars_get_input(mars_model_t *model, int index) {
    if (!model || index < 0 || (uint32_t)index >= model->header.num_inputs) return NULL;
    uint32_t tid = model->header.input_tensor_ids[index];
    if (tid >= model->header.num_tensors) return NULL;
    return &model->tensors[tid];
}

mars_runtime_tensor_t *mars_get_output(mars_model_t *model, int index) {
    if (!model || index < 0 || (uint32_t)index >= model->header.num_outputs) return NULL;
    uint32_t tid = model->header.output_tensor_ids[index];
    if (tid >= model->header.num_tensors) return NULL;
    return &model->tensors[tid];
}

int mars_get_num_inputs(mars_model_t *model) { return model ? (int)model->header.num_inputs : 0; }
int mars_get_num_outputs(mars_model_t *model) { return model ? (int)model->header.num_outputs : 0; }

void mars_print_summary(mars_model_t *model) {
    if (!model) return;
    mars_model_ext_t *m = (mars_model_ext_t *)model;
    printf("\nMars model summary (MI355X)\n");
    printf("Layers: %u\n", model->header.num_layers);
    printf("Tensors: %u\n", model->header.num_tensors);
    printf("Inputs: %u\n", model->header.num_inputs);
    printf("Outputs: %u\n", model->header.num_outputs);
    printf("Weights: %zu bytes\n", model->weights_size);
    printf("Launches per run: %d, batch %d, activations %zu bytes, parameters %zu bytes\n\n", m->n_ops, m->batch,
           m->act_bytes, m->arena_size);
}
```

thingino-accel_amd/csrc/host/mars_plan.c:

```c
#include <math.h>
#include <stdio.h>
#include <stdlib.h>
#include <string.h>
#include <time.h>

#include "mars_internal.h"
#include "nna.h"

int32_t mars_trunc_x86(float x) {
    if (x >= -2147483648.0f && x < 2147483648.0f) return (int32_t)x;
    return INT32_MIN;
}
static int sat8(int32_t v) { return v > 127 ? 127 : (v < -128 ? -128 : v); }
static int q_half_up(float v) { return sat8(mars_trunc_x86(v + 0.5f)); }

size_t elem_size(uint32_t dtype) {
    switch (dtype) {
        case MARS_DTYPE_FLOAT32: case MARS_DTYPE_INT32: return 4;
        case MARS_DTYPE_INT16: return 2;
        default: return 1;
    }
}

size_t shape_numel(const mars_tensor_t *d) {
// ... 513 lines not shown
int op_writes(const mars_op_t *o, int t) {
    if (o->t_out == t) return 1;
    for (int k = 0; k < o->chain_n; k++)
        if (o->chain_out[k] == t) return 1;
    return 0;
}

static int use_counts(const mars_model_ext_t *m, int **readers, int **writers) {
    const size_t nt = (size_t)m->pub.header.num_tensors + 1;
    int *c = (int *)calloc(2 * nt, sizeof(int));
    if (!c) return 0;
    for (int i = 0; i < m->n_ops; i++) {
        const mars_op_t *o = &m->ops[i];
        for (int k = 0; k < o->n_in; k++)
            if (o->t_in[k] >= 0) c[o->t_in[k]]++;
        if (o->t_out >= 0) c[nt + (size_t)o->t_out]++;
        for (int k = 0; k < o->chain_n; k++)
            if (o->chain_out[k] >= 0 && o->chain_out[k] != o->t_out) c[nt + (size_t)o->chain_out[k]]++;
    }
    *readers = c;
    *writers = c + nt;
    return 1;
}

static int writer_before(const mars_model_ext_t *m, int t, int before) {
    for (int k = before - 1; k >= 0; k--)
        if (m->ops[k].t_out == t) return k;
    return -1;
}

enum { USE_READ = 1, USE_WRITE = 2 };
static int touched_between(const mars_model_ext_t *m, int lo, int hi, int t, int how) {
    for (int k = lo < 0 ? 0 : lo; k < hi && k < m->n_ops; k++)
        if (((how & USE_READ) && op_reads(&m->ops[k], t)) || ((how & USE_WRITE) && op_writes(&m->ops[k], t))) return 1;
    return 0;
}
static int touched_by_other(const mars_model_ext_t *m, int t, int lo, int hi) {
    return touched_between(m, 0, lo, t, USE_READ | USE_WRITE) || touched_between(m, hi + 1, m->n_ops, t, USE_READ | USE_WRITE);
}

static void drop_dead_ops(mars_model_ext_t *m) {
    int w = 0;
    for (int i = 0; i < m->n_ops; i++)
        if (m->ops[i].kind != -1) m->ops[w++] = m->ops[i];
    m->n_ops = w;
}

size_t planned_stride(const mtensor_t *t) {
    size_t s = ALIGN_UP(t->extent > t->bytes ? t->extent : t->bytes, 256);
    return s ? s : 256;
}

static void lut2_from_lut(mars_model_ext_t *m, mars_op_t *c, const int8_t *tab) {
    if (!mhip_conv_i8_lut2_ok(c->cs)) return;
    int8_t tab2[512];
    for (int k = -256; k < 256; k++) {
        int r = k >= 0 ? (k + 1) >> 1 : -((1 - k) >> 1);
        const int lo = c->relu ? 0 : -128;
        r = r < lo ? lo : (r > 127 ? 127 : r);
        tab2[k + 256] = tab[r + 128];
    }
    c->lut2_off = arena_reserve(m, 512);
    if (c->lut2_off != NO_OFF) memcpy(m->arena_host + c->lut2_off, tab2, 512);
}

void conv_i8_geometry(const mars_op_t *op, int frames, mhip_conv_i8_t *p) {
    memset(p, 0, sizeof(*p));
    p->frames = frames;
    p->in_c = op->in_c; p->in_h = op->in_h; p->in_w = op->in_w;
    p->out_h = op->out_h; p->out_w = op->out_w; p->out_c = op->store_c ? op->store_c : op->out_c;
    p->kh = op->kh; p->kw = op->kw; p->stride_h = op->sh; p->stride_w = op->sw; p->pad_top = op->pt; p->pad_left = op->pl;
    p->row_pad = op->row_pad; p->oc_pad = op->oc_pad; p->safe = op->safe;
    p->out_pix_stride = op->out_pix_stride; p->out_ch_off = op->out_ch_off;
}
int conv_i8_pre_fits(const mars_op_t *op, int frames, size_t in_stride, size_t out_stride) {
    mhip_conv_i8_t p;
    conv_i8_geometry(op, frames, &p);
    p.in_stride = in_stride; p.out_stride = out_stride;
    p.pre_w = (const int8_t *)op; p.pre_bias = (const int32_t *)op; p.pre_lut2 = (const uint8_t *)op; p.lut2 = (const uint8_t *)op;
    p.lut = (const uint8_t *)op;
    return mhip_conv_i8_pre_ok(&p);
}

static int match_silu(const mars_model_ext_t *m, int i, int f32, const int *readers, const int *writers, int q[3], int *fwd) {
    const mars_op_t *c = &m->ops[i], *s = c + 1, *mu = c + 2;
    if (c->kind != (f32 ? OP_CONV_F32 : OP_CONV_I8) || s->kind != (f32 ? OP_SIGMOID_F32 : OP_LUT_I8) || mu->kind != (f32 ? OP_BINARY_F32 : OP_BINARY_I8) || !mu->is_mul)
        return 0;
    if (!f32 && m->pub.layers[s->layer].desc.type != MARS_LAYER_SIGMOID) return 0;
    const int q1 = q[0] = c->t_out, q2 = q[1] = s->t_out, q3 = q[2] = mu->t_out;
    if (s->t_in[0] != q1 || q1 == q2 || q2 == q3 || q1 == q3) return 0;
    *fwd = mu->t_in[0] == q1 && mu->t_in[1] == q2;
    if (!*fwd && !(mu->t_in[0] == q2 && mu->t_in[1] == q1)) return 0;
    if (f32 ? q3 == c->t_in[0] || m->mt[q3].is_weight : op_reads(c, q3)) return 0;
    if (readers[q1] != 2 || readers[q2] != 1 || writers[q1] != 1 || writers[q2] != 1 || writers[q3] != 1) return 0;
    if (m->mt[q1].io_out || m->mt[q2].io_out || m->mt[q1].io_in || m->mt[q2].io_in) return 0;
    const size_t n1 = (size_t)c->out_h * c->out_w * c->out_c;
    return s->n == n1 && mu->n == n1;
}

void fold_silu(mars_model_ext_t *m, int f32) {
    int *readers, *writers;
    if (!use_counts(m, &readers, &writers)) return;
    for (int i = 0; i + 2 < m->n_ops; i++) {
        mars_op_t *c = &m->ops[i];
        int q[3], fwd;
        if (!match_silu(m, i, f32, readers, writers, q, &fwd)) continue;
        const size_t n1 = (size_t)c->out_h * c->out_w * c->out_c;
        if (f32) {
            c->silu_f32 = 1;
        } else {
            const mars_tensor_t *d1 = &m->pub.tensors[q[0]].desc, *d2 = &m->pub.tensors[q[1]].desc, *d3 = &m->pub.tensors[q[2]].desc;
            int8_t tab[256];
            for (int v = -128; v < 128; v++) {
                int sg = sigmoid_q(v, d1->scale, d2->scale);
                tab[v + 128] = (int8_t)(fwd ? binary_q(1, v, sg, d1->scale, d2->scale, d3->scale)
                                            : binary_q(1, sg, v, d2->scale, d1->scale, d3->scale));
            }
            c->lut_off = lut_i8(m, tab);
            lut2_from_lut(m, c, tab);
        }
        c->t_out = q[2];
        touch(m, q[2], n1 * (f32 ? 4 : 1));
        m->mt[q[0]].needed = 0;
        m->mt[q[1]].needed = 0;
        memmove(&m->ops[i + 1], &m->ops[i + 3], (size_t)(m->n_ops - i - 3) * sizeof(mars_op_t));
        m->n_ops -= 2;
    }
    free(readers);
}

void fuse_lut(mars_model_ext_t *m) {
    if (m->sw.no_fuse_lut) return;
    int *readers, *writers;
    if (!use_counts(m, &readers, &writers)) return;
    for (int i = 0; i + 1 < m->n_ops; i++) {
        mars_op_t *c = &m->ops[i], *s = &m->ops[i + 1];
        if (c->kind != OP_CONV_I8 || s->kind != OP_LUT_I8 || c->lut_off != NO_OFF || s->lut_off == NO_OFF) continue;
        const int q1 = c->t_out, q2 = s->t_out;
        if (q1 < 0 || q2 < 0 || s->t_in[0] != q1 || q1 == q2) continue;
        if (op_reads(c, q2)) continue;
        if (readers[q1] != 1 || writers[q1] != 1 || writers[q2] != 1 || m->mt[q1].io_out || m->mt[q1].io_in || m->mt[q1].is_weight || m->mt[q2].is_weight) continue;
        const size_t n1 = (size_t)c->out_h * c->out_w * c->out_c;
        if (s->n != n1 || m->mt[q2].bytes < n1) continue;
        if (m->pub.tensors[q1].desc.dtype != MARS_DTYPE_INT8 || m->pub.tensors[q2].desc.dtype != MARS_DTYPE_INT8) continue;
        c->lut_off = s->lut_off;
        lut2_from_lut(m, c, (const int8_t *)(m->arena_host + s->lut_off));
        c->t_out = q2;
        touch(m, q2, n1);
        m->mt[q1].needed = 0;
        memmove(&m->ops[i + 1], &m->ops[i + 2], (size_t)(m->n_ops - i - 2) * sizeof(mars_op_t));
        m->n_ops -= 1;
    }
    free(readers);
}

void elide_concat(mars_model_ext_t *m) {
    int *readers, *writers;
    if (!use_counts(m, &readers, &writers)) return;
    for (int i = 0; i < m->n_ops; i++) {
        mars_op_t *cs = &m->ops[i];
        if (cs->kind != OP_CONCAT_SLICE) continue;
        const int ti = cs->t_in[0], to = cs->t_out;
        const mtensor_t *mt = &m->mt[ti];
        if (mt->is_weight || mt->io_in || mt->io_out || readers[ti] != 1 || writers[ti] != 1) continue;
        const int j = writer_before(m, ti, i);
        if (j < 0) continue;
// ... 262 lines not shown
            top->w2_off = NO_OFF; top->w2_rows = 0;
            mainop->t_in[0] = TL;
            mainop->in_c = CL; mainop->c_pad = CL; mainop->row_pad = row_pad2;
            mainop->in_h = mainop->out_h = H - (N - 1);
            mainop->w_off = w_off2[q];
            mainop->w2_off = NO_OFF; mainop->w2_rows = 0;
            mainop->out_byte_off = (size_t)(N - 1) * W * (size_t)mainop->out_c;
            mainop->macs = (double)(H - (N - 1)) * W * mainop->out_c * CL;
            mainop->bytes = (double)(H - (N - 1)) * W * (CL + mainop->out_c);
            mainop->variant = 0;
        }
        cq->rows_only = N - 1;
        cq->bytes = (double)(N - 1) * W * Cout * 2.0;
        m->mt[T].partial = 1;
    }
}

void fold_add(mars_model_ext_t *m, int f32) {
    int *readers, *writers;
    if (!use_counts(m, &readers, &writers)) return;
    for (int j = 0; j < m->n_ops; j++) {
        mars_op_t *ad = &m->ops[j];
        if (ad->kind != (f32 ? OP_BINARY_F32 : OP_BINARY_I8) || ad->is_mul || ad->n_in != 2 || (!f32 && ad->out_pix_stride)) continue;
        for (int side = 0; side < 2; side++) {
            const int A = ad->t_in[side], X = ad->t_in[1 - side], O = ad->t_out;
            if (A < 0 || X < 0 || O < 0 || A == X || O == X || O == A) continue;
            if (readers[A] != 1 || writers[A] != 1 || m->mt[A].io_in || m->mt[A].io_out || m->mt[A].is_weight) continue;
            if (m->mt[X].is_weight || m->mt[O].is_weight || writers[O] != 1) continue;
            const int i = writer_before(m, A, j);
            if (i < 0) continue;
            mars_op_t *c = &m->ops[i];
            if (c->kind != (f32 ? OP_CONV_F32 : OP_CONV_I8) || c->add_t || c->n_in != 1) continue;
            if (!f32 && (c->out_nchw || !c->safe || c->out_pix_stride || (c->out_c & 15) || (c->in_c & 15) || c->nseg)) continue;
            if (ad->n != (size_t)c->out_h * c->out_w * c->out_c) continue;
            if (c->t_in[0] == O) continue;
            const float s_conv = side == 0 ? ad->f0 : ad->f1, s_other = side == 0 ? ad->f1 : ad->f0, inv = ad->f2;
            if (!f32) {
                if (planned_stride(&m->mt[X]) != planned_stride(&m->mt[O])) continue;
                const double bound = 128.0 * (fabs((double)s_conv) + fabs((double)s_other)) * fabs((double)inv) + 1.0;
                if (!(bound < 2147483000.0)) continue;
            }
            if (touched_between(m, i, j + 1, X, USE_WRITE) || touched_between(m, i + 1, j, O, USE_READ | USE_WRITE)) continue;
            c->t_out = O;
            c->add_t = X + 1;
            if (!f32) { c->add_s_conv = s_conv; c->add_s_other = s_other; c->add_inv = inv; }
            c->t_in[c->n_in++] = X;
            c->bytes += (f32 ? 4.0 : 1.0) * (double)ad->n;
            m->mt[A].needed = 0;
            ad->kind = -1;
            readers[A] = 0;
            break;
        }
    }
    drop_dead_ops(m);
    free(readers);
}

void fuse_bottleneck(mars_model_ext_t *m) {
    int *readers, *writers;
    if (!use_counts(m, &readers, &writers)) return;
    for (int i = 0; i + 1 < m->n_ops; i++) {
        mars_op_t *a = &m->ops[i], *b = &m->ops[i + 1];
        if (a->kind != OP_CONV_I8 || b->kind != OP_CONV_I8 || a->pre || b->pre) continue;
        const int T = a->t_out;
        if (T < 0 || b->t_in[0] != T || readers[T] != 1 || m->mt[T].io_in || m->mt[T].io_out || m->mt[T].is_weight) continue;
        if (a->kh != 1 || a->kw != 1 || a->sh != 1 || a->sw != 1 || a->nchw || b->nchw || a->out_nchw || b->out_nchw || !a->safe || !b->safe || a->nseg || b->nseg ||
            a->add_t || a->n_in != 1 || a->out_pix_stride || a->relu || a->lut2_off == NO_OFF || b->lut2_off == NO_OFF ||
            a->in_c != a->out_c || a->out_c != b->in_c || (a->in_c != 32 && a->in_c != 64) || b->sh != 1 || b->sw != 1 ||
            a->in_h != b->in_h || a->in_w != b->in_w || a->b_off == NO_OFF || a->pair_next || b->pair_next ||
            (i > 0 && m->ops[i - 1].pair_next))
            continue;
        const int X = a->t_in[0];
        if (X < 0 || X == b->t_out || m->mt[X].is_weight) continue;
        if (!conv_i8_pre_fits(b, 1, 0, 0)) continue;
        b->pre = 1;
        b->pre_w_off = a->w_off; b->pre_b_off = a->b_off; b->pre_lut2_off = a->lut2_off; b->pre_cs = a->cs;
        b->t_in[0] = X;
        b->macs += a->macs;
        m->mt[T].needed = 0;
        readers[T] = 0;
        a->kind = -1;
    }
    drop_dead_ops(m);
    free(readers);
}

void pad_output_rows(mars_model_ext_t *m) {
    for (uint32_t i = 0; i < m->pub.header.num_tensors; i++) m->mt[i].pix_c = m->mt[i].pix_stride = 0;
    if (m->sw.no_rowpad) return;
    for (int i = 0; i < m->n_ops; i++) {
        mars_op_t *o = &m->ops[i];
        if (o->kind != OP_CONV_I8 || o->out_nchw || o->out_pix_stride || o->out_ch_off || o->add_t || o->t_out < 0 ||
            (o->out_c & 15) == 0 || (o->in_c & 15) != 0)
            continue;
        mtensor_t *t = &m->mt[o->t_out];
        const int P = (o->out_c + 15) & ~15;
        const size_t px = (size_t)o->out_h * o->out_w;
        if (!t->io_out || t->io_in || P > o->oc_pad || t->bytes != px * (size_t)o->out_c || (px * P) % 256 != 0) continue;
        if (touched_by_other(m, o->t_out, i, i)) continue;
        o->out_pix_stride = P;
        o->store_c = P;
        t->pix_c = o->out_c;
        t->pix_stride = P;
        if (px * P > t->extent) t->extent = px * P;
    }
}

void virtual_concat(mars_model_ext_t *m) {
    const int nt = (int)m->pub.header.num_tensors;
    for (int T = 0; T < nt; T++) {
        const mtensor_t *mt = &m->mt[T];
        if (mt->is_weight || mt->io_in || mt->io_out) continue;
        int sl[4], ns = 0, bad = 0, first_reader = -1, last_reader = -1, last_slice = -1;
        for (int i = 0; i < m->n_ops && !bad; i++) {
            const mars_op_t *o = &m->ops[i];
            if (o->t_out == T) {
                if (o->kind != OP_CONCAT_SLICE || ns >= 4) bad = 1;
                else { sl[ns++] = i; last_slice = i; }
            }
            for (int k = 0; k < o->n_in; k++)
                if (o->t_in[k] == T) {
                    if (o->kind != OP_CONV_I8 || k != 0 || o->n_in != 1 || o->nchw || o->kh != 1 || o->kw != 1 || o->sh != 1 ||
                        o->sw != 1 || o->pt || o->pl || !o->safe || o->nseg || (o->out_c & 15) || o->in_h != o->out_h ||
                        o->in_w != o->out_w || (o->in_c & (o->in_c - 1)) != 0 || o->add_t)
                        bad = 1;
                    if (first_reader < 0) first_reader = i;
                    last_reader = i;
                }
        }
        if (bad || ns < 2 || first_reader < 0 || last_slice > first_reader) continue;
        for (int a = 0; a < ns; a++)
            for (int b = a + 1; b < ns; b++)
                if (m->ops[sl[b]].ch_off < m->ops[sl[a]].ch_off) { int t = sl[a]; sl[a] = sl[b]; sl[b] = t; }
        int c = 0;
        const mars_op_t *s0 = &m->ops[sl[0]];
        for (int a = 0; a < ns && !bad; a++) {
            const mars_op_t *o = &m->ops[sl[a]];
            if (o->ch_off != c || (o->in_c & 31) || o->out_h != s0->out_h || o->out_w != s0->out_w || o->out_c != s0->out_c ||
                o->t_in[0] == T || o->t_in[0] < 0)
                bad = 1;
            c += o->in_c;
            if (!bad && touched_between(m, sl[a] + 1, last_reader + 1, o->t_in[0], USE_WRITE)) bad = 1;
        }
        if (bad || c != s0->out_c) continue;
        for (int i = 0; i < m->n_ops && !bad; i++) {
            const mars_op_t *o = &m->ops[i];
            if (o->kind == OP_CONV_I8 && o->n_in == 1 && o->t_in[0] == T &&
                (o->in_c != c || (size_t)o->in_h * o->in_w != (size_t)s0->out_h * s0->out_w))
                bad = 1;
        }
        if (bad) continue;
        for (int i = 0; i < m->n_ops; i++) {
            mars_op_t *o = &m->ops[i];
            if (o->kind != OP_CONV_I8 || o->n_in != 1 || o->t_in[0] != T) continue;
            o->nseg = ns;
            o->n_in = ns;
            for (int a = 0; a < ns; a++) {
                o->seg_t[a] = o->t_in[a] = m->ops[sl[a]].t_in[0];
                o->seg_c[a] = m->ops[sl[a]].in_c;
            }
        }
        for (int a = 0; a < ns; a++) m->ops[sl[a]].kind = -1;
        m->mt[T].needed = 0;
        for (int a = 0; a < ns; a++) {
            const int S = m->ops[sl[a]].t_in[0];
            int up = -1, nread = 0, nwrite = 0, ok = 1;
// ... 305 lines not shown
        }
        const int heads = 1 + paired;
        size_t wt_off[2] = {NO_OFF, NO_OFF};
        for (int q = 0; q < heads; q++) {
            const mars_op_t *x = &m->ops[r1 + q];
            wt_off[q] = arena_reserve(m, mhip_conv_f32_vcat_pack(x->out_c, x->in_c, (int)km + 1, NULL, NULL));
            if (wt_off[q] == NO_OFF) return;
            if (!m->deferred)
                mhip_conv_f32_vcat_pack(x->out_c, x->in_c, (int)km + 1, (const float *)(m->arena_host + x->w_off), (float *)(m->arena_host + wt_off[q]));
        }
        while (m->n_ops + heads > m->cap_ops) {
            const int cap = m->cap_ops * 2;
            mars_op_t *np = (mars_op_t *)realloc(m->ops, (size_t)cap * sizeof(mars_op_t));
            if (!np) { m->plan_err = MARS_ERR_ALLOC_FAILED; return; }
            m->ops = np; m->cap_ops = cap;
        }
        memmove(&m->ops[rl + 1 + heads], &m->ops[rl + 1], sizeof(mars_op_t) * (size_t)(m->n_ops - rl - 1));
        m->n_ops += heads;
        for (int q = 0; q < heads; q++) {
            mars_op_t *x = &m->ops[r1 + q], *h = &m->ops[rl + 1 + q];
            const double hw = (double)x->in_h * x->in_w;
            x->t_in[0] = TL;
            x->vc_shift = (int)sB;
            x->k_limit = (int)km;
            x->macs = hw * x->out_c * (double)km;
            x->bytes = (hw * (double)km + hw * x->out_c) * 4.0;
            *h = *x;
            h->kind = OP_CONV_F32_VHEAD;
            h->pair_next = 0; h->vc_shift = 0;
            h->k_limit = (int)km + 1;
            h->vc_n = N - 1; h->vc_run = Wb / 4;
            h->n_in = N;
            for (int k = 0; k < N - 1; k++) { h->vc_t[k] = firsts[k]; h->t_in[1 + k] = firsts[k]; }
            h->macs = (double)(sB / 4) * x->out_c * (double)(km + 1);
            h->bytes = ((double)(sB / 4) * (double)(km + 1) + (double)(sB / 4) * x->out_c) * 4.0;
            h->variant = 0;
            h->w3_off = wt_off[q]; h->w3_stem = 0;
            h->w2_off = NO_OFF; h->w2_planes = 0;
        }
        memmove(&m->ops[first_op], &m->ops[e + 1], sizeof(mars_op_t) * (size_t)(m->n_ops - e - 1));
        m->n_ops -= N;
        m->mt[T].needed = 0;
        m->mt[T].partial = 1;
        m->mt[T].zero_from = 0;
        i = first_op - 1;
    }
}

void f32_policy(mars_model_ext_t *m) {
    const int nt = (int)m->pub.header.num_tensors;
    unsigned char *hot = (unsigned char *)calloc((size_t)nt + 1, 1);
    if (!hot) {
        for (int i = 0; i < m->n_ops; i++) m->ops[i].f32_exact = 1;
        return;
    }
    for (int i = m->n_ops - 1; i >= 0; i--) {
        mars_op_t *o = &m->ops[i];
        int reach = 0;
        if (o->kind == OP_MAXPOOL && o->t_in[0] >= 0 && m->pub.tensors[o->t_in[0]].desc.dtype == MARS_DTYPE_FLOAT32) reach = 1;
        if (o->kind == OP_RELU_BYTES && o->t_out >= 0) {
            hot[o->t_out] = 1;
            continue;
        }
        if (o->t_out >= 0 && hot[o->t_out]) reach = 1;
        for (int k = 0; k < o->chain_n; k++)
            if (o->chain_out[k] >= 0 && hot[o->chain_out[k]]) reach = 1;
        if (!reach) continue;
        for (int k = 0; k < o->n_in; k++)
            if (o->t_in[k] >= 0) hot[o->t_in[k]] = 1;
        if (o->kind == OP_CONV_F32) o->f32_exact = 1;
    }
    free(hot);
}

void plan_check(mars_model_ext_t *m) {
    for (int i = 0; i < m->n_ops; i++) {
        const mars_op_t *o = &m->ops[i];
        const char *why = NULL;
        if (o->kind == -1) why = "a dead op is left";
        else if (o->n_in < 0 || o->n_in > 4 || o->nseg < 0 || o->nseg > 4 || o->chain_n < 0 || o->chain_n > 3 || o->vc_n < 0 || o->vc_n > 3) why = "an operand count is out of range";
        else if (o->add_t && !op_reads(o, o->add_t - 1)) why = "add_t is not among t_in";
        else if (o->chain_n && o->t_out != o->chain_out[o->chain_n - 1]) why = "t_out is not the chain's last stage";
        else if (o->pair_next && (i + 1 >= m->n_ops || m->ops[i + 1].kind != o->kind)) why = "pair_next without a mate of its kind";
        for (int k = 0; !why && k < o->nseg; k++)
            if (!op_reads(o, o->seg_t[k])) why = "a seg_t is not among t_in";
        for (int k = 0; !why && k < o->vc_n; k++)
            if (!op_reads(o, o->vc_t[k])) why = "a vc_t is not among t_in";
        if (!why) continue;
        VLOG("plan_check: op %d (layer %d, kind %d): %s\n", i, o->layer, o->kind, why);
        m->plan_err = MARS_ERR_LAYER_FAILED;
        return;
    }
}
```

thingino-accel_amd/csrc/host/mars_run.c:

```c
#include <math.h>
#include <stdio.h>
#include <stdlib.h>
#include <string.h>
#include <time.h>

#include "mars_internal.h"
#include "nna.h"

static int g_graph_max_batch = 8;
static unsigned g_tune_gen = 1;
static int g_dual_min_batch = 64;
static int g_dual_ways = 2;
static uint8_t *tdev(const mars_model_ext_t *m, int ti) {
    if (ti < 0 || !m->mt[ti].dev) return NULL;
    return m->mt[ti].dev + (m->mt[ti].is_weight ? 0 : (size_t)m->frame0 * m->mt[ti].stride);
}
static size_t tstride(const mars_model_ext_t *m, int ti) { return ti >= 0 ? m->mt[ti].stride : 0; }

void conv_i8_params(const mars_model_ext_t *m, const mars_op_t *op, mhip_conv_i8_t *p) {
    uint8_t *A = m->arena_dev;
    conv_i8_geometry(op, m->run_frames, p);
    p->in = (const int8_t *)tdev(m, op->t_in[0]); p->in_stride = tstride(m, op->t_in[0]);
    p->out = (int8_t *)tdev(m, op->t_out); p->out_stride = tstride(m, op->t_out);
    if (p->in) p->in += op->in_byte_off;
    if (p->out) p->out += op->out_byte_off;
    p->w = (const int8_t *)(A + op->w_off);
    p->bias = op->b_off != NO_OFF ? (const int32_t *)(A + op->b_off) : NULL;
    p->lut = op->lut_off != NO_OFF ? A + op->lut_off : NULL;
    p->lut2 = op->lut_off != NO_OFF && op->lut2_off != NO_OFF ? A + op->lut2_off : NULL;
    p->w_rgb = op->w2_off != NO_OFF && !op->w2_rows ? (const int8_t *)(A + op->w2_off) : NULL;
    p->w_rows = op->w2_off != NO_OFF && op->w2_rows ? (const int8_t *)(A + op->w2_off) : NULL;
    if (op->pre) {
        p->pre_w = (const int8_t *)(A + op->pre_w_off);
        p->pre_bias = (const int32_t *)(A + op->pre_b_off);
        p->pre_lut2 = A + op->pre_lut2_off;
        p->pre_cs = op->pre_cs;
    }
    p->cs = op->cs; p->relu = op->relu; p->out_nchw = op->out_nchw;
    p->variant = op->variant;
    if (op->add_t && tstride(m, op->add_t - 1) == p->out_stride) {
        p->add = (const int8_t *)tdev(m, op->add_t - 1);
        p->add_s_conv = op->add_s_conv; p->add_s_other = op->add_s_other; p->add_inv = op->add_inv;
    }
    p->nseg = op->nseg;
    p->seg_up = op->seg_up;
    int c0 = 0;
    for (int k = 0; k < 4; k++) {
        p->seg_c0[k] = 0x7fffffff;
        if (k < op->nseg) {
            p->seg_in[k] = (const int8_t *)tdev(m, op->seg_t[k]);
            p->seg_stride[k] = tstride(m, op->seg_t[k]);
            p->seg_c[k] = op->seg_c[k];
            p->seg_c0[k] = c0;
            c0 += op->seg_c[k];
        }
    }
    if (op->nseg > 1) p->in = p->seg_in[0];
}

static void conv_f32_params(mars_model_ext_t *m, mars_op_t *op, mhip_conv_f32_t *p) {
    const int B = m->run_frames;
    uint8_t *A = m->arena_dev;
    memset(p, 0, sizeof(*p));
    p->in = (const float *)tdev(m, op->t_in[0]); p->in_stride = tstride(m, op->t_in[0]);
    p->out = (float *)tdev(m, op->t_out); p->out_stride = tstride(m, op->t_out);
    p->w = (const float *)(A + op->w_off);
    p->w_split = op->w2_off != NO_OFF ? (const void *)(A + op->w2_off) : NULL;
    p->w_patch = op->w3_off != NO_OFF ? (const void *)(A + op->w3_off) : NULL;
    p->bias = op->b_off != NO_OFF ? (const float *)(A + op->b_off) : NULL;
    p->frames = B;
    p->in_h = op->in_h; p->in_w = op->in_w; p->in_c = op->in_c;
    p->out_h = op->out_h; p->out_w = op->out_w; p->out_c = op->out_c;
    p->kh = op->kh; p->kw = op->kw; p->stride_h = op->sh; p->stride_w = op->sw; p->pad_top = op->pt; p->pad_left = op->pl;
    p->silu = op->silu_f32;
    if (op->add_t) { p->add = (const float *)tdev(m, op->add_t - 1); p->add_stride = tstride(m, op->add_t - 1); }
    {
        const int mode = mhip_conv_f32_mode(-1);
        p->use_mfma = mode == 3 ? 3 : mode == 4 ? 2 : (mode == 2 || (mode == 1 && !op->f32_exact));
    }
    if (op->in_rec || op->out_rec) {
        p->in_rec = op->in_rec; p->out_rec = op->out_rec;
        p->use_mfma = 3;
    }
    {
        const int need = p->use_mfma == 2 ? 3 : p->use_mfma == 3 ? 2 : 0;
        if (need > op->w2_planes) p->w_split = NULL;
        if (p->use_mfma != 3) p->w_patch = NULL;
    }
    if (p->use_mfma >= 2) p->k_limit = op->k_limit;
    if (op->vc_shift && op->kind == OP_CONV_F32) {
        p->in = p->in ? (const float *)((const uint8_t *)p->in - op->vc_shift) : NULL;
        p->k_limit = op->k_limit;
        p->k_limit_required = 1;
        if (p->use_mfma < 2 || !p->w_split) p->in = NULL;
    }
}

static int launch_op(mars_model_ext_t *m, mars_op_t *op) {
    const int B = m->run_frames;
    uint8_t *A = m->arena_dev;
    switch (op->kind) {
        case OP_CONV_I8: {
            mhip_conv_i8_t p;
            conv_i8_params(m, op, &p);
            if (op->nchw && op->c_pad == 4 && op->in_c <= 4 && !op->add_t) {
                if (!getenv("MARS_HIP_NO_PLANAR_STEM")) {
                    mhip_conv_i8_t q = p;
                    q.in_c = op->c_pad;
                    q.in_planar = op->in_c;
                    const int rc = mhip_conv_i8(&q);
                    if (rc != -2) return rc;
                }
            }
            if (op->nchw) {
                const size_t ss = ALIGN_UP(m->scratch_per_frame, 256);
                int8_t *scratch = (int8_t *)m->scratch_dev + (size_t)m->frame0 * ss;
                if (!(m->scratch_t == op->t_in[0] && m->scratch_cpad == op->c_pad && m->scratch_f0 == m->frame0 && m->scratch_n == B)) {
                    int rc = mhip_nchw_to_nhwc_pad(p.in, p.in_stride, scratch, ss, B, op->in_c, op->in_h * op->in_w, op->c_pad);
                    if (rc) return rc;
                    m->scratch_t = op->t_in[0]; m->scratch_cpad = op->c_pad; m->scratch_f0 = m->frame0; m->scratch_n = B;
                }
                p.in = scratch; p.in_stride = ss; p.in_c = op->c_pad;
            }
            if (op->add_t && !p.add) return -1;
            return mhip_conv_i8(&p);
        }
        case OP_CONV_F32: {
            mhip_conv_f32_t p;
            conv_f32_params(m, op, &p);
            return mhip_conv_f32(&p);
        }
        case OP_CONV_F32_VHEAD: {
            mhip_conv_f32_t p;
            const float *first[3] = {NULL, NULL, NULL};
            size_t strides[3] = {0, 0, 0};
            conv_f32_params(m, op, &p);
            if (p.use_mfma < 2) return -1;
            p.k_limit = op->k_limit;
            for (int k = 0; k < op->vc_n && k < 3; k++) {
                first[k] = (const float *)tdev(m, op->vc_t[k]);
// ... 80 lines not shown
                                    op->out_h, op->out_w, op->scale_h, op->scale_w, op->out_pix_stride, op->out_ch_off);
        default: return -1;
    }
}

static mars_error_t enqueue_plan(mars_model_t *model);
static double now_us(void);
static int tune_raw(const char *key, int value, int *get);

static void tune_push(mars_model_ext_t *m) {
    if (m->tune_depth++ || !m->n_tune) return;
    for (int i = 0; i < m->n_tune; i++) {
        tune_raw(m->tune[i].key, 0, &m->tune[i].saved);
        tune_raw(m->tune[i].key, m->tune[i].value, NULL);
    }
}
static void tune_pop(mars_model_ext_t *m) {
    if (--m->tune_depth || !m->n_tune) return;
    for (int i = m->n_tune - 1; i >= 0; i--) tune_raw(m->tune[i].key, m->tune[i].saved, NULL);
}
static mars_error_t run_device_async(mars_model_t *model);
mars_error_t mars_hip_run_device_async(mars_model_t *model) {
    if (!model) return MARS_ERR_INVALID_FILE;
    tune_push((mars_model_ext_t *)model);
    mars_error_t e = run_device_async(model);
    tune_pop((mars_model_ext_t *)model);
    return e;
}

static mars_error_t run_device_async(mars_model_t *model) {
    mars_model_ext_t *m = (mars_model_ext_t *)model;
    if (!m->act_dev || !m->arena_dev) return MARS_ERR_NNA_INIT_FAILED;
    int graphable = g_graph_max_batch > 0 && m->batch <= g_graph_max_batch && !m->profiling && !m->pipe;
    for (int i = 0; i < m->n_ops && graphable; i++)
        if (m->ops[i].kind == OP_FAIL) graphable = 0;
    if (!graphable) return enqueue_plan(model);
    if (m->graph_exec && m->graph_gen != g_tune_gen) {
        drop_graph(m);
        m->ran_plain = 0;
    }
    if (!m->graph_exec) {
        if (!m->ran_plain) {
            mars_error_t e = enqueue_plan(model);
            if (e == MARS_OK) m->ran_plain = 1;
            return e;
        }
        if (m->tail_pending) {
            mhip_select_stream(0);
            if (mhip_stream_wait(0, m->ev_tail_done)) return MARS_ERR_LAYER_FAILED;
            m->tail_pending = 0;
        }
        if (mhip_graph_begin() == 0) {
            mars_error_t e = enqueue_plan(model);
            m->graph_exec = mhip_graph_end(e == MARS_OK);
            m->graph_gen = g_tune_gen;
            if (e != MARS_OK) { m->graph_exec = NULL; return e; }
        }
        VLOG("plan of %d launches at batch %d %s\n", m->n_ops, m->batch, m->graph_exec ? "captured into a HIP graph" : "could not be captured");
        if (!m->graph_exec) {
            g_graph_max_batch = 0;
            return enqueue_plan(model);
        }
    }
    if (m->tail_pending) {
        mhip_select_stream(0);
        if (mhip_stream_wait(0, m->ev_tail_done)) return MARS_ERR_LAYER_FAILED;
        m->tail_pending = 0;
    }
    if (mhip_graph_launch(m->graph_exec)) return MARS_ERR_LAYER_FAILED;
    for (uint32_t i = 0; i < model->header.num_layers; i++) model->layers[i].is_executed = true;
    return MARS_OK;
}

static mars_error_t enqueue_range(mars_model_ext_t *m, int sid, int wait_tail) {
    void *prof_last = NULL;
    mhip_select_stream(sid);
    m->scratch_t = -1;
    for (int i = 0; i < m->n_ops; i++) {
        mars_op_t *op = &m->ops[i];
        if (op->kind == OP_FAIL) {
            fprintf(stderr, "Mars: Layer %d execution failed\n", op->layer);
            return (mars_error_t)op->err;
        }
        mars_op_t *mate = op->pair_next && i + 1 < m->n_ops ? &m->ops[i + 1] : NULL;
        if (wait_tail && ((op->t_out >= 0 && (m->mt[op->t_out].io_out || m->mt[op->t_out].tail_read)) ||
                          (mate && mate->t_out >= 0 && (m->mt[mate->t_out].io_out || m->mt[mate->t_out].tail_read)))) {
            mhip_stream_wait(sid, m->ev_tail_done);
            wait_tail = 0;
        }
        if (m->profiling) {
            if (!op->ev1) op->ev1 = mhip_event_create();
            if (!prof_last) {
                if (!op->ev0) op->ev0 = mhip_event_create();
                mhip_event_record(op->ev0);
                prof_last = op->ev0;
            }
            op->ev_start = prof_last;
        }
        int rc;
        if (mate && op->kind == OP_CONV_F32) {
            mhip_conv_f32_t pa, pb;
            conv_f32_params(m, op, &pa);
            conv_f32_params(m, mate, &pb);
            rc = mhip_conv_f32_pair(&pa, &pb);
            if (rc == -2) {
                rc = launch_op(m, op);
                if (!rc) rc = launch_op(m, mate);
            }
            i++;
        } else if (mate) {
            mhip_conv_i8_t pa, pb;
            conv_i8_params(m, op, &pa);
            conv_i8_params(m, mate, &pb);
            rc = mhip_conv_i8_pair(&pa, &pb);
            if (rc == -2) {
                rc = launch_op(m, op);
                if (!rc) rc = launch_op(m, mate);
            }
            i++;
        } else {
            rc = launch_op(m, op);
        }
        {
            const mars_op_t *w2[2] = {op, mate};
            for (int q = 0; q < 2; q++)
                if (w2[q] && op_writes(w2[q], m->scratch_t)) m->scratch_t = -1;
        }
        if (m->profiling) {
            const int nx = i + 1;
            const int end = m->profiling != 2 || nx >= m->n_ops || m->ops[nx].prof_kind != op->prof_kind;
            op->prof_rec = end;
            if (end) {
                mhip_event_record(op->ev1);
                prof_last = op->ev1;
            }
        }
        if (rc != 0) {
            fprintf(stderr, "Mars: Layer %d launch failed: %s\n", op->layer, mhip_last_error());
            return MARS_ERR_LAYER_FAILED;
        }
    }
    return MARS_OK;
}

static mars_error_t enqueue_plan(mars_model_t *model) {
    mars_model_ext_t *m = (mars_model_ext_t *)model;
    for (uint32_t i = 0; i < model->header.num_layers; i++) model->layers[i].is_executed = false;
    const int B = m->batch;
    int dual = g_dual_min_batch > 0 && B >= g_dual_min_batch && B >= 2 && !m->profiling &&
               !(g_graph_max_batch > 0 && B <= g_graph_max_batch);
    if (dual) {
        if (!m->ev_fork) m->ev_fork = mhip_event_create_sync();
        for (int k = 0; k < 3; k++) {
            if (!m->ev_join[k]) m->ev_join[k] = mhip_event_create_sync();
            if (!m->ev_join[k]) dual = 0;
        }
        if (!m->ev_fork) dual = 0;
    }
    mars_error_t e;
    if (!dual) {
        m->frame0 = 0; m->run_frames = B;
        e = enqueue_range(m, 0, m->tail_pending);
    } else {
        const int ways = g_dual_ways < B ? g_dual_ways : B;
        mhip_select_stream(0);
        int rc = mhip_event_record(m->ev_fork);
        for (int k = 1; k < ways && !rc; k++) rc = mhip_stream_wait(3 + k, m->ev_fork);
        if (rc) return MARS_ERR_LAYER_FAILED;
        e = MARS_OK;
        int f0 = 0;
        for (int k = 0; k < ways && e == MARS_OK; k++) {
            const int n = (B - f0 + (ways - k) - 1) / (ways - k);
            m->frame0 = f0; m->run_frames = n;
            e = enqueue_range(m, k ? 3 + k : 0, m->tail_pending);
            f0 += n;
        }
        for (int k = 1; k < ways; k++) {
            mhip_select_stream(3 + k);
            rc = mhip_event_record(m->ev_join[k - 1]);
            if (!rc) rc = mhip_stream_wait(0, m->ev_join[k - 1]);
            if (rc && e == MARS_OK) e = MARS_ERR_LAYER_FAILED;
        }
    }
// ... 198 lines not shown
        if (value < 0 || value > 4) return -1;
        mhip_conv_f32_mode(value);
        return 0;
    }
    return get ? mhip_conv_i8_tune_get(key, get) : mhip_conv_i8_tune(key, value);
}

static mars_error_t replan_for_f32_mode(mars_model_ext_t *m) {
    if (m->deferred || !m->arena_dev) return MARS_OK;
    int has_f32 = 0;
    for (int i = 0; i < m->n_ops && !has_f32; i++) has_f32 = m->ops[i].kind == OP_CONV_F32;
    if (!has_f32) return MARS_OK;
    tune_push(m);
    const int mode = mhip_conv_f32_mode(-1);
    mars_error_t e = MARS_OK;
    if (mode != m->plan_f32_mode && (mode >= 3 || m->plan_f32_mode >= 3)) {
        mhip_sync();
        e = build_plan(m);
        if (e == MARS_OK) e = upload_params(m);
        if (e == MARS_OK) e = alloc_batch(m, m->batch > 0 ? m->batch : 1);
    }
    tune_pop(m);
    return e;
}

int mars_hip_set_tuning(const char *key, int value) {
    g_tune_gen++;
    int rc = tune_raw(key, value, NULL);
    if (rc == 0 && key && !strcmp(key, "f32_mfma"))
        for (mars_model_ext_t *m = mars_live_models(); m; m = m->live_next)
            if (replan_for_f32_mode(m) != MARS_OK) rc = -1;
    return rc;
}

int mars_hip_get_tuning(const char *key, int *value) { return value ? tune_raw(key, 0, value) : -1; }

int mars_hip_model_set_tuning(mars_model_t *model, const char *key, int value) {
    mars_model_ext_t *m = (mars_model_ext_t *)model;
    int cur;
    if (!m || !key || strlen(key) >= sizeof m->tune[0].key || tune_raw(key, 0, &cur)) return -1;
    if (tune_raw(key, value, NULL)) return -1;
    tune_raw(key, cur, NULL);
    int i = 0;
    while (i < m->n_tune && strcmp(m->tune[i].key, key)) i++;
    if (i == m->n_tune) {
        if (m->n_tune == MARS_MAX_MODEL_TUNE) return -1;
        strcpy(m->tune[m->n_tune++].key, key);
    }
    m->tune[i].value = value;
    drop_graph(m);
    if (!strcmp(key, "f32_mfma") && replan_for_f32_mode(m) != MARS_OK) return -1;
    return 0;
}

int mars_hip_model_get_tuning(mars_model_t *model, const char *key, int *value) {
    mars_model_ext_t *m = (mars_model_ext_t *)model;
    if (!m || !key || !value) return -1;
    for (int i = 0; i < m->n_tune; i++)
        if (!strcmp(m->tune[i].key, key)) { *value = m->tune[i].value; return 0; }
    return tune_raw(key, 0, value);
}

static mars_error_t autotune_model(mars_model_t *model, int reps);
mars_error_t mars_hip_autotune(mars_model_t *model, int reps) {
    if (!model) return MARS_ERR_INVALID_FILE;
    tune_push((mars_model_ext_t *)model);
    mars_error_t e = autotune_model(model, reps);
    tune_pop((mars_model_ext_t *)model);
    return e;
}
static mars_error_t autotune_model(mars_model_t *model, int reps) {
    mars_model_ext_t *m = (mars_model_ext_t *)model;
    if (!m->act_dev || !m->arena_dev) return MARS_ERR_NNA_INIT_FAILED;
    drop_graph(m);
    if (reps <= 0) reps = 3;
    void *e0 = mhip_event_create(), *e1 = mhip_event_create();
    if (!e0 || !e1) return MARS_ERR_ALLOC_FAILED;
    mars_error_t err = MARS_OK;
    if (mhip_sync()) err = MARS_ERR_LAYER_FAILED;
    for (int i = 0; i < m->n_ops && err == MARS_OK; i++) {
        mars_op_t *op = &m->ops[i];
        if (op->kind != OP_CONV_I8 || op->nchw) continue;
        if (op->pair_next || (i > 0 && m->ops[i - 1].pair_next)) continue;
        mhip_conv_i8_t p;
        conv_i8_params(m, op, &p);
        int codes[32];
        const int n = mhip_conv_i8_variants(&p, codes, 32);
        if (getenv("MARS_VERBOSE") && atoi(getenv("MARS_VERBOSE")) > 1)
            fprintf(stderr, "Mars: autotune layer %d: %dx%dx%d -> %dx%dx%d k%dx%d s%d pixstride %d choff %d lut %d safe %d\n", op->layer,
                    p.in_h, p.in_w, p.in_c, p.out_h, p.out_w, p.out_c, p.kh, p.kw, p.stride_w, p.out_pix_stride, p.out_ch_off,
                    p.lut != NULL, p.safe);
        float best = 0.0f;
        int best_code = 0;
        for (int k = 0; k < n && err == MARS_OK; k++) {
            p.variant = codes[k];
            int rc = mhip_conv_i8(&p);
            if (!rc) rc = mhip_event_record(e0);
            for (int r = 0; r < reps && !rc; r++) rc = mhip_conv_i8(&p);
            if (!rc) rc = mhip_event_record(e1);
            if (rc || mhip_sync()) { err = MARS_ERR_LAYER_FAILED; break; }
            const float ms = mhip_event_elapsed_ms(e0, e1);
            if (getenv("MARS_VERBOSE") && atoi(getenv("MARS_VERBOSE")) > 1)
                fprintf(stderr, "Mars: autotune layer %d: candidate %d: %.1f us\n", op->layer, codes[k], ms * 1000.0f / reps);
            if (best_code == 0 || ms < best) { best = ms; best_code = codes[k]; }
        }
        if (err == MARS_OK && best_code) {
            if (getenv("MARS_VERBOSE"))
                fprintf(stderr, "Mars: autotune layer %d: variant %d (%.1f us) of %d candidates, default %d\n", op->layer,
                        best_code, best * 1000.0f / reps, n, n ? codes[0] : 0);
            op->variant = best_code;
        }
    }
    mhip_event_destroy(e0);
    mhip_event_destroy(e1);
    return err;
}

void *mars_hip_tensor_device(mars_model_t *model, int ti, size_t *frame_stride) {
    if (!model || ti < 0 || (uint32_t)ti >= model->header.num_tensors) return NULL;
    mars_model_ext_t *m = (mars_model_ext_t *)model;
    if (frame_stride) *frame_stride = m->mt[ti].stride;
    return m->mt[ti].dev;
}

size_t mars_hip_tensor_frame_bytes(const mars_model_t *model, int ti) {
    if (!model || ti < 0 || (uint32_t)ti >= model->header.num_tensors) return 0;
    return ((const mars_model_ext_t *)model)->mt[ti].bytes;
}

int mars_hip_tensor_row_pitch(mars_model_t *model, int ti, int *row_bytes) {
    if (!model || ti < 0 || (uint32_t)ti >= model->header.num_tensors) return 0;
    const mtensor_t *t = &((mars_model_ext_t *)model)->mt[ti];
    if (row_bytes) *row_bytes = t->pix_stride ? t->pix_c : 0;
    return t->pix_stride;
}

mars_error_t mars_hip_read_tensor(mars_model_t *model, int ti, int frame, void *dst, size_t bytes) {
    if (!model || !dst || ti < 0 || (uint32_t)ti >= model->header.num_tensors) return MARS_ERR_INVALID_TENSOR;
    mars_model_ext_t *m = (mars_model_ext_t *)model;
    mtensor_t *t = &m->mt[ti];
    if (!t->dev || frame < 0 || (!t->is_weight && frame >= m->batch)) return MARS_ERR_INVALID_TENSOR;
    if (!t->is_weight && bytes > t->stride) return MARS_ERR_INVALID_TENSOR;
    if (t->partial) return MARS_ERR_INVALID_TENSOR;
    if (t->is_weight) {
        const size_t off = (size_t)m->pub.tensors[ti].desc.data_offset;
        if (off > m->blob_mirror_bytes || bytes > m->blob_mirror_bytes - off) return MARS_ERR_INVALID_TENSOR;
        frame = 0;
    }
    if (mhip_sync()) return MARS_ERR_LAYER_FAILED;
    if (t->rec_c) {
        const size_t full = (size_t)t->rec_c * t->rec_hw * 4;
        uint8_t *raw = (uint8_t *)malloc(full);
        float *f = (float *)malloc(full);
        if (!raw || !f || bytes > full || mhip_d2h_async(raw, t->dev + (size_t)frame * t->stride, full) || mhip_sync()) {
            free(raw); free(f);
            return MARS_ERR_LAYER_FAILED;
        }
        for (int c = 0; c < t->rec_c; c++)
            for (int px = 0; px < t->rec_hw; px++) {
                const uint8_t *r = raw + ((size_t)(c >> 3) * t->rec_hw + px) * 32 + (size_t)(c & 7) * 2;
                uint16_t h, md;
                memcpy(&h, r, 2); memcpy(&md, r + 16, 2);
                const uint32_t hb = (uint32_t)h << 16, mb = (uint32_t)md << 16;
                float hf, mf;
                memcpy(&hf, &hb, 4); memcpy(&mf, &mb, 4);
                f[(size_t)c * t->rec_hw + px] = hf + mf;
// ... 120 lines not shown
```

thingino-accel_amd/csrc/mhip.h:

```cpp
#ifndef MHIP_H
#define MHIP_H

#include <stddef.h>
#include <stdint.h>

#ifdef __cplusplus
extern "C" {
#endif

int mhip_init(int device_hint);
void mhip_shutdown(void);
int mhip_ready(void);
int mhip_device_info(int *cu_count, int *lds_bytes, int *gfx_version, size_t *hbm_bytes);
void *mhip_stream(void);
int mhip_sync(void);
void mhip_select_aux(int on);
void mhip_select_stream(int which);
int mhip_stream_wait(int which, void *ev);
int mhip_event_sync(void *ev);
void *mhip_malloc(size_t bytes);
void mhip_free(void *p);
void *mhip_host_alloc(size_t bytes);
void mhip_host_free(void *p);
int mhip_memset_async(void *dst, int value, size_t bytes);
int mhip_h2d_async(void *dst, const void *src, size_t bytes);
int mhip_d2h_async(void *dst, const void *src, size_t bytes);
int mhip_d2d_async(void *dst, const void *src, size_t bytes);
int mhip_h2d_2d_async(void *dst, size_t dpitch, const void *src, size_t spitch, size_t row_bytes, size_t rows);
int mhip_d2h_2d_async(void *dst, size_t dpitch, const void *src, size_t spitch, size_t row_bytes, size_t rows);
void *mhip_event_create(void);
void *mhip_event_create_sync(void);
void mhip_event_destroy(void *ev);
int mhip_event_record(void *ev);
float mhip_event_elapsed_ms(void *start, void *stop);
const char *mhip_last_error(void);
int mhip_graph_begin(void);
void *mhip_graph_end(int ok);
int mhip_graph_launch(void *exec);
void mhip_graph_destroy(void *exec);

typedef struct {
    const int8_t *in;  size_t in_stride;
    int8_t *out;       size_t out_stride;
    const int8_t *w;
    const int32_t *bias;
    const uint8_t *lut;
    const uint8_t *lut2;
    const int8_t *pre_w;
    const int32_t *pre_bias;
    const uint8_t *pre_lut2;
    float pre_cs;
    const int8_t *w_rgb;
    const int8_t *w_rows;
    int frames;
    int in_h, in_w, in_c;
    int out_h, out_w, out_c;
    int kh, kw, stride_h, stride_w, pad_top, pad_left;
    int row_pad;
    int oc_pad;
    float cs;
    int relu;
    int out_nchw;
    int in_planar;
    int safe;
    int out_pix_stride;
    int out_ch_off;
    int variant;
    const int8_t *add;
    float add_s_conv, add_s_other, add_inv;
    int nseg;
    const int8_t *seg_in[4];
    size_t seg_stride[4];
    int seg_c[4], seg_c0[4];
    int seg_up;
} mhip_conv_i8_t;
int mhip_conv_i8_oc_row(int oc, int oc_pad);
int mhip_conv_i8_pre_ok(const mhip_conv_i8_t *p);
size_t mhip_conv_i8_rgb_pack(int in_c, int kh, int kw, int stride_h, int stride_w, int pad_left, int oc_pad, int k64,
                             const int8_t *packed, int8_t *out);
size_t mhip_conv_i8_rows_pack(int in_c, int kh, int kw, int stride_h, int stride_w, int oc_pad, int k64, int out_w,
                              const int8_t *packed, int8_t *out);
unsigned long mhip_conv_i8_rows_launches(void);
int mhip_conv_i8_is_safe(float cs);
int mhip_conv_i8_lut2_ok(float cs);
int mhip_conv_i8_tune(const char *key, int value);
int mhip_conv_i8_tune_get(const char *key, int *value);
int mhip_conv_i8_variants(const mhip_conv_i8_t *p, int *codes, int max);
int mhip_conv_i8_seg_ok(const mhip_conv_i8_t *p);
int mhip_conv_i8_pair(const mhip_conv_i8_t *a, const mhip_conv_i8_t *b);
int mhip_conv_i8_small_c(int in_c, int kw, int out_c);
void mhip_conv_i8_pack_geom(int in_c, int kw, int out_c, int *row_pad, int *oc_pad, int *c_eff);
int mhip_conv_i8(const mhip_conv_i8_t *p);

typedef struct {
    const float *in;  size_t in_stride;
    float *out;       size_t out_stride;
    const float *w;   const float *bias;
    const void *w_split;
    const void *w_patch;
    int frames;
    int in_h, in_w, in_c, out_h, out_w, out_c;
    int kh, kw, stride_h, stride_w, pad_top, pad_left;
    int silu;
    const float *add; size_t add_stride;
    int use_mfma;
    int k_limit;
    int k_limit_required;
    int in_rec, out_rec;
} mhip_conv_f32_t;
int mhip_conv_f32(const mhip_conv_f32_t *p);
size_t mhip_conv_f32_vcat_pack(int out_c, int in_c, int planes, const float *w, float *out);
int mhip_conv_f32_vcat_head(const mhip_conv_f32_t *p, const float *w_t, const float *const *first, const size_t *first_strides, int n_first, int run_floats);
int mhip_conv_f32_pair(const mhip_conv_f32_t *a, const mhip_conv_f32_t *b);
unsigned long mhip_conv_f32_pair_launches(void);
size_t mhip_conv_f32_split_pack(int out_c, int in_c, int kh, int kw, int stride_w, int planes, const float *w, void *out);
unsigned long mhip_conv_f32_split_launches(void);
int mhip_conv_f32_split_takes(int out_c, int in_c, int kh, int kw, int stride_h, int stride_w, int pad_left, int in_w, int out_w);
size_t mhip_conv_f32_patch_pack(int out_c, int in_c, int kh, int kw, int stride, int pad, int in_h, int in_w, int out_h, int out_w,
                                const float *w, void *out);
size_t mhip_conv_f32_patch_pack2(int out_c, int in_c, int kh, int kw, int stride, int pad, int in_h, int in_w, int out_h, int out_w,
                                 int rec, const float *w, void *out);
int mhip_conv_f32_patch_geom2(int out_c, int in_c, int kh, int kw, int stride, int pad, int in_h, int in_w, int out_h, int out_w,
                              int rec, int *outv, int cap);
unsigned long mhip_conv_f32_prec_launches(void);
unsigned long mhip_conv_f32_recin_launches(void);
int mhip_conv_f32_patch_rec_form(int out_c, int in_c, int kh, int kw, int stride, int pad, int in_h, int in_w, int out_h, int out_w);
int mhip_conv_f32_patch_geom(int out_c, int in_c, int kh, int kw, int stride, int pad, int in_h, int in_w, int out_h, int out_w,
                             int *outv, int cap);
unsigned long mhip_conv_f32_patch_launches(void);
size_t mhip_conv_f32_stem_pack(int out_c, int in_c, int kh, int kw, int stride, int pad, int in_h, int in_w, int out_h, int out_w,
                               const float *w, void *out);
unsigned long mhip_conv_f32_stem_launches(void);
int mhip_conv_f32_mode(int set);

int mhip_lut_i8(const int8_t *in, size_t in_stride, int8_t *out, size_t out_stride, int frames,
                size_t n, const uint8_t *lut_dev);
int mhip_relu_bytes(int8_t *buf, size_t stride, int frames, size_t n);
int mhip_binary_i8(int is_mul, const int8_t *a, size_t a_stride, const int8_t *b, size_t b_stride,
                   int8_t *out, size_t out_stride, int frames, size_t n, float sa, float sb, float inv_so,
                   int out_run, int out_pix_stride, int out_ch_off);
int mhip_sigmoid_f32(const float *in, size_t in_stride, float *out, size_t out_stride, int frames, size_t n);
int mhip_binary_f32(int op , const float *a, size_t a_stride, const float *b,
                    size_t b_stride, float *out, size_t out_stride, int frames, size_t n);
int mhip_relu_f32(const float *in, size_t in_stride, float *out, size_t out_stride, int frames,
                  size_t n, float alpha);
int mhip_batchnorm_i8(const int8_t *in, size_t in_stride, int8_t *out, size_t out_stride, int frames,
                      int n, int c, int hw, const float *s, const float *b, float in_scale, float out_scale);
int mhip_batchnorm_f32(const float *in, size_t in_stride, float *out, size_t out_stride, int frames,
                       int n, int c, int hw, const float *s, const float *b);

int mhip_maxpool_i8(const int8_t *in, size_t in_stride, int8_t *out, size_t out_stride, int frames,
                    int in_h, int in_w, int ch, int out_h, int out_w, int kh, int kw, int sh, int sw,
                    int out_pix_stride, int out_ch_off);
int mhip_pool_chain_i8(const int8_t *in, size_t in_stride, int8_t *const *outs, const size_t *out_strides, int n,
                       int frames, int h, int w, int ch, int kh, int kw);
int mhip_unpad_rows(const void *src, void *dst, size_t rows, int width, int pitch);
int mhip_concat_slice(const int8_t *in, size_t in_stride, int8_t *out, size_t out_stride, int frames,
                      int out_h, int out_w, int in_c, int out_c, int ch_off);
// ... 205 lines not shown
```

Before: 56820.

## Fuse trailing C3 cv3 1x1 concat conv into the preceding 3x3 patch conv epilogue

Adds a POST mode to the patch conv kernel. It takes the requantized output of a 3x3 conv, stages the second concat input (y2) into LDS, and runs the following 1x1 conv over the concatenated 2c channels with in-register MFMAs before storing the final result. The planner pass fuse_post detects the conv pair and packs the 1x1 weights and bias into a special layout. The intermediate tensor is never written to or read back from memory, and one kernel launch is removed. In exchange the kernel uses more LDS and registers, which may lower occupancy or force smaller tiles.

Result: faster. 57640 (median of 6 runs) (+1.4%).

```diff
diff --git a/thingino-accel_amd/csrc/hip/conv_i8.hip b/thingino-accel_amd/csrc/hip/conv_i8.hip
--- a/thingino-accel_amd/csrc/hip/conv_i8.hip
+++ b/thingino-accel_amd/csrc/hip/conv_i8.hip
@@ -1140,6 +1140,11 @@
             }
         return n;
     }
+    if (p->post_w) {
+        for (int th : {16, 8, 4})
+            if (n < max && conv_i8_patch_ok(p, th, nullptr)) codes[n++] = th == 16 ? 10 : (th == 8 ? 9 : 11);
+        return n;
+    }
     if (p->nseg > 1) {
         const int bn = p->oc_pad % 128 == 0 ? 128 : (p->oc_pad % 64 == 0 ? 64 : 32);
         const variant_t dv = default_variant(p, nks);
@@ -1182,7 +1187,7 @@
 }
 
 extern "C" int mhip_conv_i8(const mhip_conv_i8_t *p) {
-    if (!p || !p->in || !p->out || !p->w) return -1;
+    if (!p || !p->in || (!p->out && !(p->post_w && p->post_out)) || !p->w) return -1;
     if (p->out_pix_stride < 0 || p->out_ch_off < 0 || (p->out_nchw && (p->out_pix_stride || p->out_ch_off)) ||
         (p->out_pix_stride && p->out_pix_stride < p->out_ch_off + p->out_c))
         return -1;
@@ -1227,6 +1232,19 @@
         }
         return conv_i8_launch_patch(p, k64, th);
     }
+    if (p->post_w) {
+        if (!mhip_zero_page() || (p->in_c % 16) != 0 || !mhip_conv_i8_post_ok(p)) return -1;
+        int th = conv_i8_post_tile_rows(p);
+        const int code = p->variant ? p->variant : tune().variant;
+        if (code >= 9 && code <= 11) {
+            const int want = code == 10 ? 16 : (code == 9 ? 8 : 4);
+            if (conv_i8_patch_ok(p, want, nullptr)) th = want;
+        } else if (tune().small_batch && conv_i8_patch_ok(p, 4, nullptr) &&
+                   ((long)p->frames * p->out_h * p->out_w + 255) / 256 * ((p->oc_pad + 127) / 128) < tune().few_wgs) {
+            th = 4;
+        }
+        return conv_i8_launch_patch(p, k64, th);
+    }
     if ((p->in_c % 16) == 0) {
         if (!mhip_zero_page()) return -1;
         const int nks = k64 / BK;
diff --git a/thingino-accel_amd/csrc/hip/conv_i8_common.hpp b/thingino-accel_amd/csrc/hip/conv_i8_common.hpp
--- a/thingino-accel_amd/csrc/hip/conv_i8_common.hpp
+++ b/thingino-accel_amd/csrc/hip/conv_i8_common.hpp
@@ -424,6 +424,7 @@
 bool conv_i8_patch_ok(const mhip_conv_i8_t *p, int th, int *ring);
 int conv_i8_launch_patch(const mhip_conv_i8_t *p, int k64, int th);
 int conv_i8_pre_tile_rows(const mhip_conv_i8_t *p);
+int conv_i8_post_tile_rows(const mhip_conv_i8_t *p);
 bool conv_i8_rows_ok(const mhip_conv_i8_t *p);
 int conv_i8_launch_rows(const mhip_conv_i8_t *p);
 int conv_i8_try_rgb(const mhip_conv_i8_t *p, int k64);
diff --git a/thingino-accel_amd/csrc/hip/conv_i8_patch.hip b/thingino-accel_amd/csrc/hip/conv_i8_patch.hip
--- a/thingino-accel_amd/csrc/hip/conv_i8_patch.hip
+++ b/thingino-accel_amd/csrc/hip/conv_i8_patch.hip
@@ -41,7 +41,7 @@
     asm volatile("s_waitcnt lgkmcnt(0)\n\ts_barrier" ::: "memory");
 }
 
-template <int TH, int BN, bool HAS_LUT, bool PRE = false>
+template <int TH, int BN, bool HAS_LUT, bool PRE = false, bool POST = false>
 __global__ __launch_bounds__(NTHREADS) void conv_i8_patch(const mhip_conv_i8_t p, const int k64, const int tiles_x,
                                                           const int tiles_y, const unsigned ntiles_all, const int PH,
                                                           const int PW, const int PWP, const int PWH, const int nblk,
@@ -56,12 +56,15 @@
     uint8_t *slut = (uint8_t *)dynlds;
     lds_base_must_be_zero(dynlds);
     const int nks = k64 / BK;
-    constexpr int LB = LUTB + (PRE ? 512 : 0);
+    constexpr int NPO = 2 * BN;
+    constexpr int LB = LUTB + ((PRE || POST) ? 512 : 0);
     int *dutab = (int *)(dynlds + LB);
     int8_t *wl = dynlds + LB + ((nks * 16 + 255) & ~255);
     const int patch_bytes = nblk * 1024;
     int8_t *w1l = wl + nks * BN * BK;
-    int8_t *patch0 = w1l + (PRE ? p.in_c * BK : 0);
+    int8_t *pwl = w1l;
+    const int *pbl = (const int *)(pwl + NPO * NPO);
+    int8_t *patch0 = w1l + (PRE ? p.in_c * BK : 0) + (POST ? NPO * NPO + NPO * 4 : 0);
     int8_t *tpatch = patch0 + ring * patch_bytes;
 
     const int tid = threadIdx.x, lane = tid & 63;
@@ -85,6 +88,10 @@
         else if (tid < 64) ((uint32_t *)slut)[tid] = ((const uint32_t *)p.lut)[tid];
     }
     if (PRE && tid >= 128) ((uint32_t *)slut)[tid] = ((const uint32_t *)p.pre_lut2)[tid - 128];
+    if (POST) {
+        if (tid >= 128) ((uint32_t *)slut)[tid] = ((const uint32_t *)p.post_lut2)[tid - 128];
+        if (tid < NPO) ((int *)(pwl + NPO * NPO))[tid] = ((const int *)(p.post_w + NPO * NPO))[tid];
+    }
     const int rowbytes = p.kw * C, kbytes = p.kh * rowbytes;
     for (int i = tid; i < nks * 4; i += NTHREADS) {
         const int kb = i * 16;
@@ -105,6 +112,8 @@
         }
         if (PRE)
             for (int g = wv; g < C / 16; g += 4) glds16(p.pre_w + (size_t)(g * 16 + (lane >> 2)) * BK + schunk * 16, w1l + g * 16 * BK);
+        if (POST)
+            for (int i = wv; i < NPO * NPO / 1024; i += 4) glds16(p.post_w + i * 1024 + lane * 16, pwl + i * 1024);
     }
     int uoff[PT_NIMAX], upos[PT_NIMAX];
 #pragma unroll
@@ -160,14 +169,31 @@
             }
     };
 
-    const __amdgpu_buffer_rsrc_t orsrc = __builtin_amdgcn_make_buffer_rsrc(p.out, 0, (int)out_bytes, 0x00020000);
+    const __amdgpu_buffer_rsrc_t orsrc = __builtin_amdgcn_make_buffer_rsrc(POST ? p.post_out : p.out, 0, (int)out_bytes, 0x00020000);
     const bool has_add = p.add != nullptr;
     constexpr int RROW = WOC == 4 ? 1024 : 512;
     constexpr int NRI = WOC == 4 ? WPX : 2 * WPX;
     int8_t *rstage = patch0 + (ring + (PRE ? 1 : 0)) * patch_bytes + wv * (WPX * RROW);
-    const int NR = has_add ? NRI : 0;
     const int frow = lane & 15, fchunk = lane >> 4;
     const int chan = (lane >> 4) * (4 * WOC);
+    const int NR = has_add || POST ? NRI : 0;
+    const int ntail = POST ? (has_add ? NRI : 0) + WPX * (NPO / 64) : NST;
+    const int ppstride = p.post_out_pix_stride ? p.post_out_pix_stride : NPO;
+    auto issue_rows = [&](const int8_t *base, size_t fstride, int tx, int ty, unsigned f) {
+#pragma unroll
+        for (int u = 0; u < WPX; u++) {
+            const int oy = ty * TH + wv * WPX + u, ox = tx * PT_TW + frow;
+            const int8_t *src = oy < p.out_h && ox < p.out_w ? base + (size_t)f * fstride + ((size_t)(oy * p.out_w + ox) * BN + (size_t)chan) : zeros;
+            if (WOC == 4) {
+                glds16(src, rstage + u * RROW);
+            } else {
+                __builtin_amdgcn_global_load_lds((const __attribute__((address_space(1))) void *)src,
+                                                 (__attribute__((address_space(3))) void *)(rstage + u * RROW), 4, 0, 0);
+                __builtin_amdgcn_global_load_lds((const __attribute__((address_space(1))) void *)(src + 4),
+                                                 (__attribute__((address_space(3))) void *)(rstage + u * RROW + 256), 4, 0, 0);
+            }
+        }
+    };
     const int pstride = p.out_pix_stride ? p.out_pix_stride : p.out_c;
     const int lo = p.relu ? 0 : -128;
     const uint8_t *lut128 = slut + 128;
@@ -214,7 +240,17 @@
 #pragma unroll
             for (int q = 0; q < WOC; q++) xw[u][q] = 0;
         }
-        if (has_add) {
+        if (POST) {
+#pragma unroll
+            for (int u = 0; u < WPX; u++) {
+                const int oy = ty * TH + wv * WPX + u, ox = tx * PT_TW + frow;
+                const unsigned off = f * (unsigned)p.post_out_stride + (unsigned)(oy * p.out_w + ox) * (unsigned)ppstride +
+                                     (unsigned)(p.post_out_ch_off + (lane >> 4) * (NPO / 4));
+                voffs[u] = oy < p.out_h && ox < p.out_w ? (int)off : -1;
+            }
+            if (has_add) issue_rows(p.add, p.out_stride, tx, ty, f);
+            else issue_rows(p.post_in, p.post_in_stride, tx, ty, f);
+        } else if (has_add) {
 #pragma unroll
             for (int u = 0; u < WPX; u++) {
                 const int8_t *src = voffs[u] >= 0 ? p.add + (unsigned)voffs[u] : zeros;
@@ -240,12 +276,12 @@
                 issue_patch(tn, patch0 + slot * patch_bytes);
                 pn = npw;
             }
-            const int after = NR + pn + NST;
+            const int after = NR + pn + ntail;
             yg0 = yg1 + after;
             yg1 = yg2 + after;
-            yg2 = NST;
-            if (D == 1) yg0 = NST;
-            if (D == 2) yg1 = NST;
+            yg2 = ntail;
+            if (D == 1) yg0 = ntail;
+            if (D == 2) yg1 = ntail;
             pn_last = pn;
         } else {
             if (!first) barrier_lds();
@@ -361,6 +397,15 @@
                 }
             }
         }
+        uint32_t pku[POST ? WPX : 1][WOC];
+        if (POST && has_add) {
+#pragma unroll
+            for (int u = 0; u < WPX; u++) {
+                if constexpr (WOC == 4) asm volatile("s_waitcnt lgkmcnt(0)" : "+v"(xw[u][0]), "+v"(xw[u][1]), "+v"(xw[u][2]), "+v"(xw[u][3])::"memory");
+                else asm volatile("s_waitcnt lgkmcnt(0)" : "+v"(xw[u][0]), "+v"(xw[u][1])::"memory");
+            }
+            issue_rows(p.post_in, p.post_in_stride, tx, ty, f);
+        }
 #pragma unroll
         for (int u = 0; u < WPX; u++) {
             uint32_t pk[WOC];
@@ -378,11 +423,48 @@
                 if (fast) requant_pack<WOC * 4, HAS_LUT, true, true, false, true>(a, p.cs, lo, lut128, pk);
                 else requant_pack<WOC * 4, HAS_LUT, true, true>(a, p.cs, lo, lut128, pk);
             }
+            if (POST) {
+#pragma unroll
+                for (int q = 0; q < WOC; q++) pku[POST ? u : 0][q] = pk[q];
+                continue;
+            }
             const int voff = voffs[u];
             if (WOC == 4)
                 __builtin_amdgcn_raw_buffer_store_b128((v4i){(int)pk[0], (int)pk[1], (int)pk[2], (int)pk[3]}, orsrc, voff, 0, 0);
             else if (WOC == 2)
                 __builtin_amdgcn_raw_buffer_store_b64((v2i){(int)pk[0], (int)pk[WOC > 1 ? 1 : 0]}, orsrc, voff, 0, 0);
+        }
+        if (POST) {
+            if (has_add) wait_vmcnt<0>();
+            else if (D > 0) wait_vmcnt_upto<15>(pn_last);
+#pragma unroll
+            for (int u = 0; u < WPX; u++) {
+                v4i b0, b1 = {0, 0, 0, 0};
+                if (WOC == 4) {
+                    b0 = (v4i){(int)pku[POST ? u : 0][0], (int)pku[POST ? u : 0][1], (int)pku[POST ? u : 0][WOC > 2 ? 2 : 0], (int)pku[POST ? u : 0][WOC > 3 ? 3 : 0]};
+                    b1 = *(const v4i *)(rstage + u * RROW + lane * 16);
+                } else {
+                    b0 = (v4i){(int)pku[POST ? u : 0][0], (int)pku[POST ? u : 0][WOC > 1 ? 1 : 0], *(const int *)(rstage + u * RROW + lane * 4),
+                               *(const int *)(rstage + u * RROW + 256 + lane * 4)};
+                }
+#pragma unroll
+                for (int h = 0; h < NPO / 64; h++) {
+                    int a[16];
+#pragma unroll
+                    for (int s4 = 0; s4 < 4; s4++) {
+                        const int row = (h * 4 + s4) * 16;
+                        v4i c = *(const v4i *)(pbl + row + fchunk * 4);
+                        c = __builtin_amdgcn_mfma_i32_16x16x64_i8(*(const v4i *)(pwl + lds_off(row + frow, fchunk)), b0, c, 0, 0, 0);
+                        if (WOC == 4) c = __builtin_amdgcn_mfma_i32_16x16x64_i8(*(const v4i *)(pwl + NPO * BK + lds_off(row + frow, fchunk)), b1, c, 0, 0, 0);
+#pragma unroll
+                        for (int e = 0; e < 4; e++) a[s4 * 4 + e] = c[e];
+                    }
+                    uint32_t pk4[4];
+                    requant_pack_pre<16>(a, p.post_cs, pk4);
+                    const int voff = voffs[u] >= 0 ? voffs[u] + h * 16 : -1;
+                    __builtin_amdgcn_raw_buffer_store_b128((v4i){(int)pk4[0], (int)pk4[1], (int)pk4[2], (int)pk4[3]}, orsrc, voff, 0, 0);
+                }
+            }
         }
 #ifdef PATCH_STAMPS
         STAMP(st4);
@@ -433,10 +515,19 @@
     if (g->nblk > 4 * PT_NIMAX) return false;
     const bool pre = p->pre_w != nullptr;
     if (pre && (s != 1 || (C != 32 && C != 64) || !p->pre_bias || !p->pre_lut2 || !p->lut2)) return false;
+    const bool post = p->post_w != nullptr;
+    if (post) {
+        const long ppstride = p->post_out_pix_stride ? p->post_out_pix_stride : 2 * g->bn;
+        if (pre || s != 1 || p->out_c != g->bn || p->oc_pad != g->bn || p->out_pix_stride || p->out_ch_off || !p->lut2 || !p->post_lut2 || !p->post_in ||
+            !p->post_out || ((p->post_out_pix_stride | p->post_out_ch_off) & 15) || p->post_out_pix_stride < 0 || p->post_out_ch_off < 0 ||
+            ppstride < p->post_out_ch_off + 2 * g->bn ||
+            (long)(p->frames - 1) * (long)p->post_out_stride + (long)p->out_h * p->out_w * ppstride > 0x7fffffffL)
+            return false;
+    }
     const size_t pb = (size_t)g->nblk * 1024;
-    const size_t radd = p->add ? (size_t)4 * (th / 4) * (g->bn == 64 ? 1024 : 512) : 0;
-    const size_t fixed = LUTB + (pre ? 512 + (size_t)C * BK + pb : 0) + (((size_t)g->nks * 16 + 255) & ~(size_t)255) +
-                         (size_t)g->nks * g->bn * BK + radd;
+    const size_t radd = p->add || post ? (size_t)4 * (th / 4) * (g->bn == 64 ? 1024 : 512) : 0;
+    const size_t fixed = LUTB + (pre ? 512 + (size_t)C * BK + pb : 0) + (post ? 512 + (size_t)4 * g->bn * g->bn + (size_t)8 * g->bn : 0) +
+                         (((size_t)g->nks * 16 + 255) & ~(size_t)255) + (size_t)g->nks * g->bn * BK + radd;
     const size_t budget = patch_lds_budget(g->bn);
     if (fixed + pb > budget) return false;
     const int fit = (int)((budget - fixed) / pb);
@@ -448,9 +539,13 @@
     return true;
 }
 
-template <int TH, int BN, bool HAS_LUT, bool PRE = false>
+static inline long post_out_bytes(const mhip_conv_i8_t *p) {
+    const long ppstride = p->post_out_pix_stride ? p->post_out_pix_stride : 2 * p->out_c;
+    return (long)(p->frames - 1) * (long)p->post_out_stride + (long)p->out_h * p->out_w * ppstride;
+}
+template <int TH, int BN, bool HAS_LUT, bool PRE = false, bool POST = false>
 static int launch_patch_t(const mhip_conv_i8_t *p, int k64, const patch_geom_t &g) {
-    auto kern = conv_i8_patch<TH, BN, HAS_LUT, PRE>;
+    auto kern = conv_i8_patch<TH, BN, HAS_LUT, PRE, POST>;
     static int cus = 0;
     static size_t slots_lds[8];
     static int slots_n[8], nslots = 0;
@@ -493,7 +588,7 @@
     hipLaunchKernelGGL(kern, dim3(gx, noc), dim3(NTHREADS), g.lds, mhip_stream_native(), *p, k64,
                        g.tiles_x, g.tiles_y, ntiles, g.PH, g.PW, g.PWP, g.PWH, g.nblk, (const int8_t *)mhip_zero_page(),
                        make_fastdiv((unsigned)g.tiles_x), make_fastdiv((unsigned)g.tiles_y), make_fastdiv((unsigned)g.PWP),
-                       (unsigned)persist_out_bytes(p), g.ring, xmap,
+                       (unsigned)(POST ? post_out_bytes(p) : persist_out_bytes(p)), g.ring, xmap,
                        in_extent_bytes(p) <= 0x7fffffffL ? (unsigned)in_extent_bytes(p) : 0u);
     return mhip_check(hipGetLastError(), "conv_i8_patch launch");
 }
@@ -509,8 +604,9 @@
     patch_geom_t g;
     if (!patch_geom(p, th, &g)) return -1;
 #define PATCH(T, B)                                                                       \
-    (p->pre_w ? launch_patch_t<T, B, true, true>(p, k64, g)                               \
-              : (p->lut ? launch_patch_t<T, B, true>(p, k64, g) : launch_patch_t<T, B, false>(p, k64, g)))
+    (p->post_w ? launch_patch_t<T, B, true, false, true>(p, k64, g)                       \
+     : p->pre_w ? launch_patch_t<T, B, true, true>(p, k64, g)                             \
+                : (p->lut ? launch_patch_t<T, B, true>(p, k64, g) : launch_patch_t<T, B, false>(p, k64, g)))
     if (th == 16) return g.bn == 64 ? PATCH(16, 64) : PATCH(16, 32);
     if (th == 8) return g.bn == 64 ? PATCH(8, 64) : PATCH(8, 32);
     return g.bn == 64 ? PATCH(4, 64) : PATCH(4, 32);
@@ -527,3 +623,38 @@
     if (!p || !p->pre_w || p->nseg > 1 || p->out_nchw) return 0;
     return conv_i8_pre_tile_rows(p) != 0;
 }
+
+int conv_i8_post_tile_rows(const mhip_conv_i8_t *p) {
+    patch_geom_t g;
+    for (int th : {16, 8, 4})
+        if (patch_geom(p, th, &g)) return th;
+    return 0;
+}
+extern "C" int mhip_conv_i8_post_ok(const mhip_conv_i8_t *p) {
+    if (!p || !p->post_w || p->pre_w || p->nseg > 1 || p->out_nchw) return 0;
+    return conv_i8_post_tile_rows(p) != 0;
+}
+extern "C" int mhip_conv_i8_post_k(int c, int k) {
+    if (c == 64) return k;
+    return k < 32 ? (k >> 3) * 16 + (k & 7) : ((k - 32) >> 3) * 16 + 8 + (k & 7);
+}
+extern "C" int mhip_conv_i8_post_row(int c, int oc) {
+    const int per = c / 2, g = oc / per, rem = oc - g * per;
+    return (rem >> 2) * 16 + g * 4 + (rem & 3);
+}
+extern "C" size_t mhip_conv_i8_post_pack(int c, const int8_t *packed, const int32_t *bias, int8_t *out) {
+    if (c != 32 && c != 64) return 0;
+    const int n = 2 * c;
+    const size_t bytes = (size_t)n * n + (size_t)n * 4;
+    if (!packed || !out) return bytes;
+    memset(out, 0, bytes);
+    for (int oc = 0; oc < n; oc++) {
+        const int R = mhip_conv_i8_post_row(c, oc), src = mhip_conv_i8_oc_row(oc, n);
+        for (int k = 0; k < n; k++) {
+            const int pos = mhip_conv_i8_post_k(c, k), ks = pos >> 6, chunk = (pos & 63) >> 4;
+            out[(size_t)(ks * n + R) * BK + (((chunk ^ ((R >> 1) & 2))) << 4) + (pos & 15)] = packed[(size_t)src * n + k];
+        }
+        ((int32_t *)(out + (size_t)n * n))[R] = bias ? bias[src] : 0;
+    }
+    return bytes;
+}
diff --git a/thingino-accel_amd/csrc/host/mars_internal.h b/thingino-accel_amd/csrc/host/mars_internal.h
--- a/thingino-accel_amd/csrc/host/mars_internal.h
+++ b/thingino-accel_amd/csrc/host/mars_internal.h
@@ -77,6 +77,8 @@
     int pre;
     size_t pre_w_off, pre_b_off, pre_lut2_off;
     float pre_cs;
+    int post_next;
+    size_t post_w_off;
     size_t w2_off;
     int w2_rows;
     int w2_planes;
@@ -96,7 +98,7 @@
 typedef struct {
     int fusion;
     unsigned no_fuse_lut : 1, no_nhwc_internal : 1, no_vconcat_q : 1, no_pair_f32 : 1, no_rec : 1, no_zero_tail : 1, no_vconcat_f32 : 1,
-        no_rowpad : 1;
+        no_rowpad : 1, no_post : 1;
     size_t rec_limit;
     size_t vconcat_limit;
     size_t bottleneck_limit;
@@ -110,6 +112,7 @@
     int no_vconcat;
     int no_download;
     int no_bottleneck;
+    int no_post;
     int rec_frames;
     int rec_skipped;
     size_t rec_max_frames;
@@ -207,6 +210,7 @@
 MARS_INTERNAL size_t planned_stride(const mtensor_t *t);
 MARS_INTERNAL void conv_i8_geometry(const mars_op_t *op, int frames, mhip_conv_i8_t *p);
 MARS_INTERNAL int conv_i8_pre_fits(const mars_op_t *op, int frames, size_t in_stride, size_t out_stride);
+MARS_INTERNAL int conv_i8_post_fits(const mars_model_ext_t *m, const mars_op_t *a, const mars_op_t *b, int frames);
 MARS_INTERNAL void plan_layer(mars_model_ext_t *m, int li);
 MARS_INTERNAL void fold_silu(mars_model_ext_t *m, int f32);
 MARS_INTERNAL void fuse_lut(mars_model_ext_t *m);
@@ -218,6 +222,7 @@
 MARS_INTERNAL void fuse_pool_chains(mars_model_ext_t *m);
 MARS_INTERNAL void pair_convs(mars_model_ext_t *m);
 MARS_INTERNAL void fuse_bottleneck(mars_model_ext_t *m);
+MARS_INTERNAL void fuse_post(mars_model_ext_t *m);
 MARS_INTERNAL void pad_output_rows(mars_model_ext_t *m);
 MARS_INTERNAL void virtual_concat_q(mars_model_ext_t *m);
 MARS_INTERNAL void f32_policy(mars_model_ext_t *m);
diff --git a/thingino-accel_amd/csrc/host/mars_model.c b/thingino-accel_amd/csrc/host/mars_model.c
--- a/thingino-accel_amd/csrc/host/mars_model.c
+++ b/thingino-accel_amd/csrc/host/mars_model.c
@@ -26,6 +26,7 @@
     sw->no_zero_tail = getenv("MARS_HIP_NO_ZERO_TAIL") != NULL;
     sw->no_vconcat_f32 = getenv("MARS_HIP_NO_VCONCAT_F32") != NULL;
     sw->no_rowpad = getenv("MARS_HIP_NO_ROWPAD") != NULL;
+    sw->no_post = getenv("MARS_HIP_NO_POST") != NULL;
     sw->rec_limit = (e = getenv("MARS_HIP_REC_LIMIT")) ? (size_t)strtoull(e, NULL, 0) : (size_t)0xfffffff0u;
     sw->vconcat_limit = (e = getenv("MARS_HIP_VCONCAT_LIMIT")) ? (size_t)strtoull(e, NULL, 0) : (size_t)0x7fffffffu;
     sw->bottleneck_limit = (e = getenv("MARS_HIP_BOTTLENECK_LIMIT")) ? (size_t)strtoull(e, NULL, 0) : 0;
@@ -158,6 +159,7 @@
         fuse_pool_chains(m);
         pair_convs(m);
         if (m->sw.fusion >= 2 && !m->no_bottleneck) fuse_bottleneck(m);
+        fuse_post(m);
         pad_output_rows(m);
         virtual_concat_q(m);
     } else {
@@ -199,8 +201,8 @@
     const size_t vlim = m->sw.vconcat_limit, blim = m->sw.bottleneck_limit;
     const int rec_replan = (size_t)n > m->rec_max_frames || (m->rec_skipped && n < m->rec_frames);
     m->rec_frames = n;
-    if (m->no_vconcat || m->no_bottleneck || rec_replan) {
-        m->no_vconcat = m->no_bottleneck = 0;
+    if (m->no_vconcat || m->no_bottleneck || m->no_post || rec_replan) {
+        m->no_vconcat = m->no_bottleneck = m->no_post = 0;
         mars_error_t e = build_plan(m);
         if (e == MARS_OK) e = upload_params(m);
         if (e != MARS_OK) return e;
@@ -224,6 +226,18 @@
             const size_t in_stride = op->t_in[0] >= 0 ? planned_stride(&m->mt[op->t_in[0]]) : 0;
             if (!conv_i8_pre_fits(op, n, in_stride, planned_stride(&m->mt[op->t_out])) || (blim && (size_t)n > blim)) {
                 m->no_bottleneck = 1;
+                mars_error_t e = build_plan(m);
+                if (e == MARS_OK) e = upload_params(m);
+                if (e != MARS_OK) return e;
+                break;
+            }
+        }
+    if (!m->no_post)
+        for (int i = 0; i + 1 < m->n_ops; i++) {
+            const mars_op_t *op = &m->ops[i];
+            if (op->kind != OP_CONV_I8 || !op->post_next) continue;
+            if (!conv_i8_post_fits(m, op, op + 1, n)) {
+                m->no_post = 1;
                 mars_error_t e = build_plan(m);
                 if (e == MARS_OK) e = upload_params(m);
                 if (e != MARS_OK) return e;
@@ -380,6 +394,8 @@
     ADD(" w_off %zd b_off %zd lut_off %zd lut2_off %zd s_off %zd w2_off %zd rows %d planes %d w3_off %zd stem %d blob %zd %zd", (ssize_t)o->w_off, (ssize_t)o->b_off,
         (ssize_t)o->lut_off, (ssize_t)o->lut2_off, (ssize_t)o->s_off, (ssize_t)o->w2_off, o->w2_rows, o->w2_planes, (ssize_t)o->w3_off, o->w3_stem, (ssize_t)o->w_blob_off[0],
         (ssize_t)o->w_blob_off[1]);
+    ADD(" post_next %d", o->post_next);
+    if (o->post_next) ADD(" %zd", (ssize_t)o->post_w_off);
     ADD(" pre %d", o->pre);
     if (o->pre) ADD(" %zd %zd %zd %a", (ssize_t)o->pre_w_off, (ssize_t)o->pre_b_off, (ssize_t)o->pre_lut2_off, (double)o->pre_cs);
     ADD(" macs %a bytes %a prof_kind %d", o->macs, o->bytes, o->prof_kind);
@@ -404,7 +420,7 @@
 #define FLAG(cond, ...) if (cond) k += snprintf(line + k, sizeof line - (size_t)k, __VA_ARGS__)
         FLAG(o->kind == OP_CONV_I8 || o->kind == OP_CONV_F32 || o->kind == OP_CONV_F32_VHEAD, " k%dx%d s%d c%d->%d", o->kh, o->kw, o->sw, o->in_c, o->out_c);
         FLAG(o->nchw, " relayout"); FLAG(o->out_nchw, " planar_store"); FLAG(o->lut_off != NO_OFF, " lut"); FLAG(o->add_t, " add=%d", o->add_t - 1);
-        FLAG(o->nseg, " seg=%d", o->nseg); FLAG(o->pair_next, " pair_next"); FLAG(o->pre, " pre"); FLAG(o->silu_f32, " silu");
+        FLAG(o->nseg, " seg=%d", o->nseg); FLAG(o->pair_next, " pair_next"); FLAG(o->post_next, " post_next"); FLAG(o->pre, " pre"); FLAG(o->silu_f32, " silu");
         FLAG(o->k_limit, " k_limit=%d", o->k_limit); FLAG(o->in_rec, " in_rec=%d", o->in_rec); FLAG(o->out_rec, " out_rec");
         FLAG(o->vc_shift, " view=-%d", o->vc_shift); FLAG(o->vc_n, " vcat=%dx%d", o->vc_n, o->vc_run);
         FLAG(o->rows_only, " rows_only=%d", o->rows_only); FLAG(o->out_byte_off, " out_off=%zu", o->out_byte_off); FLAG(o->chain_n, " chain=%d", o->chain_n);
@@ -430,10 +446,10 @@
     if (full) {
         const plan_switches_t *w = &m->sw;
         snprintf(line, sizeof line, "+plan n_ops %d arena_size %zu scratch_per_frame %zu blob_mirror_bytes %zu rec_max_frames %zu rec_skipped %d f32_mode %d | fusion %d"
-                 " no_fuse_lut %d no_nhwc_internal %d no_vconcat_q %d no_pair_f32 %d no_rec %d no_zero_tail %d no_vconcat_f32 %d no_rowpad %d rec_limit %zu"
+                 " no_fuse_lut %d no_nhwc_internal %d no_vconcat_q %d no_pair_f32 %d no_rec %d no_zero_tail %d no_vconcat_f32 %d no_rowpad %d no_post %d rec_limit %zu"
                  " vconcat_limit %zu bottleneck_limit %zu\n", m->n_ops, m->arena_size, m->scratch_per_frame, m->blob_mirror_bytes, m->rec_max_frames, m->rec_skipped,
                  m->plan_f32_mode, w->fusion, w->no_fuse_lut, w->no_nhwc_internal, w->no_vconcat_q, w->no_pair_f32, w->no_rec, w->no_zero_tail, w->no_vconcat_f32,
-                 w->no_rowpad, w->rec_limit, w->vconcat_limit, w->bottleneck_limit);
+                 w->no_rowpad, w->no_post, w->rec_limit, w->vconcat_limit, w->bottleneck_limit);
         EMIT();
     }
 #undef EMIT
diff --git a/thingino-accel_amd/csrc/host/mars_plan.c b/thingino-accel_amd/csrc/host/mars_plan.c
--- a/thingino-accel_amd/csrc/host/mars_plan.c
+++ b/thingino-accel_amd/csrc/host/mars_plan.c
@@ -619,6 +619,19 @@
     return mhip_conv_i8_pre_ok(&p);
 }
 
+int conv_i8_post_fits(const mars_model_ext_t *m, const mars_op_t *a, const mars_op_t *b, int frames) {
+    mhip_conv_i8_t p;
+    if (a->t_in[0] < 0 || a->t_out < 0 || b->t_out < 0) return 0;
+    conv_i8_geometry(a, frames, &p);
+    p.in_stride = planned_stride(&m->mt[a->t_in[0]]); p.out_stride = planned_stride(&m->mt[a->t_out]);
+    p.lut = p.lut2 = p.post_lut2 = (const uint8_t *)a;
+    p.post_w = p.post_in = (const int8_t *)a; p.post_out = (int8_t *)m;
+    if (a->add_t) p.add = (const int8_t *)a;
+    p.post_out_stride = planned_stride(&m->mt[b->t_out]);
+    p.post_out_pix_stride = b->out_pix_stride; p.post_out_ch_off = b->out_ch_off;
+    return mhip_conv_i8_post_ok(&p);
+}
+
 static int match_silu(const mars_model_ext_t *m, int i, int f32, const int *readers, const int *writers, int q[3], int *fwd) {
     const mars_op_t *c = &m->ops[i], *s = c + 1, *mu = c + 2;
     if (c->kind != (f32 ? OP_CONV_F32 : OP_CONV_I8) || s->kind != (f32 ? OP_SIGMOID_F32 : OP_LUT_I8) || mu->kind != (f32 ? OP_BINARY_F32 : OP_BINARY_I8) || !mu->is_mul)
@@ -1047,6 +1060,47 @@
         a->kind = -1;
     }
     drop_dead_ops(m);
+    free(readers);
+}
+
+void fuse_post(mars_model_ext_t *m) {
+    if (m->sw.no_post || m->no_post) return;
+    int *readers, *writers;
+    if (!use_counts(m, &readers, &writers)) return;
+    for (int i = 0; i + 1 < m->n_ops; i++) {
+        mars_op_t *a = &m->ops[i], *b = &m->ops[i + 1];
+        if (a->kind != OP_CONV_I8 || b->kind != OP_CONV_I8 || a->pre || b->pre || a->post_next || b->post_next || a->pair_next || b->pair_next ||
+            (i > 0 && (m->ops[i - 1].pair_next || m->ops[i - 1].post_next)))
+            continue;
+        const int c = a->out_c, T = a->t_out, O = b->t_out;
+        if ((c != 32 && c != 64) || a->oc_pad != c || a->kh * a->kw < 2 || a->sh != 1 || a->sw != 1 || !a->safe || a->nchw || a->out_nchw || a->nseg ||
+            a->out_pix_stride || a->out_ch_off || a->store_c || a->chain_n || a->in_byte_off || a->out_byte_off || a->lut_off == NO_OFF ||
+            a->lut2_off == NO_OFF || a->n_in >= 4)
+            continue;
+        if (b->kh != 1 || b->kw != 1 || b->sh != 1 || b->sw != 1 || b->pt || b->pl || !b->safe || b->nchw || b->out_nchw || b->add_t || b->chain_n ||
+            b->store_c || b->in_byte_off || b->lut_off == NO_OFF || b->lut2_off == NO_OFF || b->nseg != 2 || b->seg_up || b->seg_t[0] != T ||
+            b->seg_c[0] != c || b->seg_c[1] != c || b->in_c != 2 * c || b->out_c != 2 * c || b->oc_pad != 2 * c || b->row_pad != 2 * c ||
+            b->in_h != a->out_h || b->in_w != a->out_w || b->out_h != a->out_h || b->out_w != a->out_w)
+            continue;
+        const int Y = b->seg_t[1];
+        if (T < 0 || O < 0 || Y < 0 || Y == T || O == T || O == Y || readers[T] != 1 || writers[T] != 1 || m->mt[T].io_in || m->mt[T].io_out ||
+            m->mt[T].is_weight || m->mt[T].tail_read || m->mt[Y].is_weight || m->mt[Y].pix_stride ||
+            m->mt[Y].bytes != (size_t)a->out_h * a->out_w * c || op_reads(a, O) || op_reads(a, Y))
+            continue;
+        if (!conv_i8_post_fits(m, a, b, 1)) continue;
+        const size_t bytes = mhip_conv_i8_post_pack(c, NULL, NULL, NULL);
+        const size_t off = arena_reserve(m, bytes);
+        if (off == NO_OFF) break;
+        mhip_conv_i8_post_pack(c, (const int8_t *)(m->arena_host + b->w_off), b->b_off != NO_OFF ? (const int32_t *)(m->arena_host + b->b_off) : NULL,
+                               (int8_t *)(m->arena_host + off));
+        a->post_next = 1;
+        a->post_w_off = off;
+        a->t_in[a->n_in++] = Y;
+        m->mt[T].needed = 0;
+        readers[T] = 0;
+        readers[Y]++;
+        i++;
+    }
     free(readers);
 }
 
@@ -1518,6 +1572,9 @@
         else if (o->add_t && !op_reads(o, o->add_t - 1)) why = "add_t is not among t_in";
         else if (o->chain_n && o->t_out != o->chain_out[o->chain_n - 1]) why = "t_out is not the chain's last stage";
         else if (o->pair_next && (i + 1 >= m->n_ops || m->ops[i + 1].kind != o->kind)) why = "pair_next without a mate of its kind";
+        else if (o->post_next && (o->kind != OP_CONV_I8 || i + 1 >= m->n_ops || m->ops[i + 1].kind != OP_CONV_I8 || m->ops[i + 1].nseg != 2 ||
+                                  m->ops[i + 1].seg_t[0] != o->t_out || !op_reads(o, m->ops[i + 1].seg_t[1])))
+            why = "post_next without its 1x1 behind it, or y2 is not among t_in";
         for (int k = 0; !why && k < o->nseg; k++)
             if (!op_reads(o, o->seg_t[k])) why = "a seg_t is not among t_in";
         for (int k = 0; !why && k < o->vc_n; k++)
diff --git a/thingino-accel_amd/csrc/host/mars_run.c b/thingino-accel_amd/csrc/host/mars_run.c
--- a/thingino-accel_amd/csrc/host/mars_run.c
+++ b/thingino-accel_amd/csrc/host/mars_run.c
@@ -38,6 +38,7 @@
     }
     p->cs = op->cs; p->relu = op->relu; p->out_nchw = op->out_nchw;
     p->variant = op->variant;
+    if (op->post_next && op->t_out >= 0) p->out_stride = planned_stride(&m->mt[op->t_out]);
     if (op->add_t && tstride(m, op->add_t - 1) == p->out_stride) {
         p->add = (const int8_t *)tdev(m, op->add_t - 1);
         p->add_s_conv = op->add_s_conv; p->add_s_other = op->add_s_other; p->add_inv = op->add_inv;
@@ -56,6 +57,18 @@
         }
     }
     if (op->nseg > 1) p->in = p->seg_in[0];
+}
+
+static void conv_i8_post_params(const mars_model_ext_t *m, const mars_op_t *op, const mars_op_t *cv3, mhip_conv_i8_t *p) {
+    uint8_t *A = m->arena_dev;
+    conv_i8_params(m, op, p);
+    p->post_w = (const int8_t *)(A + op->post_w_off);
+    p->post_lut2 = A + cv3->lut2_off;
+    p->post_cs = cv3->cs;
+    p->post_in = (const int8_t *)tdev(m, cv3->seg_t[1]); p->post_in_stride = tstride(m, cv3->seg_t[1]);
+    p->post_out = (int8_t *)tdev(m, cv3->t_out); p->post_out_stride = tstride(m, cv3->t_out);
+    if (p->post_out) p->post_out += cv3->out_byte_off;
+    p->post_out_pix_stride = cv3->out_pix_stride; p->post_out_ch_off = cv3->out_ch_off;
 }
 
 static void conv_f32_params(mars_model_ext_t *m, mars_op_t *op, mhip_conv_f32_t *p) {
@@ -302,7 +315,7 @@
             fprintf(stderr, "Mars: Layer %d execution failed\n", op->layer);
             return (mars_error_t)op->err;
         }
-        mars_op_t *mate = op->pair_next && i + 1 < m->n_ops ? &m->ops[i + 1] : NULL;
+        mars_op_t *mate = (op->pair_next || op->post_next) && i + 1 < m->n_ops ? &m->ops[i + 1] : NULL;
         if (wait_tail && ((op->t_out >= 0 && (m->mt[op->t_out].io_out || m->mt[op->t_out].tail_read)) ||
                           (mate && mate->t_out >= 0 && (m->mt[mate->t_out].io_out || m->mt[mate->t_out].tail_read)))) {
             mhip_stream_wait(sid, m->ev_tail_done);
@@ -318,7 +331,12 @@
             op->ev_start = prof_last;
         }
         int rc;
-        if (mate && op->kind == OP_CONV_F32) {
+        if (mate && op->post_next) {
+            mhip_conv_i8_t pa;
+            conv_i8_post_params(m, op, mate, &pa);
+            rc = mhip_conv_i8(&pa);
+            i++;
+        } else if (mate && op->kind == OP_CONV_F32) {
             mhip_conv_f32_t pa, pb;
             conv_f32_params(m, op, &pa);
             conv_f32_params(m, mate, &pb);
@@ -683,6 +701,7 @@
         mars_op_t *op = &m->ops[i];
         if (op->kind != OP_CONV_I8 || op->nchw) continue;
         if (op->pair_next || (i > 0 && m->ops[i - 1].pair_next)) continue;
+        if (op->post_next || (i > 0 && m->ops[i - 1].post_next)) continue;
         mhip_conv_i8_t p;
         conv_i8_params(m, op, &p);
         int codes[32];
diff --git a/thingino-accel_amd/csrc/mhip.h b/thingino-accel_amd/csrc/mhip.h
--- a/thingino-accel_amd/csrc/mhip.h
+++ b/thingino-accel_amd/csrc/mhip.h
@@ -73,7 +73,17 @@
     size_t seg_stride[4];
     int seg_c[4], seg_c0[4];
     int seg_up;
+    const int8_t *post_w;
+    const uint8_t *post_lut2;
+    float post_cs;
+    const int8_t *post_in;  size_t post_in_stride;
+    int8_t *post_out;       size_t post_out_stride;
+    int post_out_pix_stride, post_out_ch_off;
 } mhip_conv_i8_t;
+int mhip_conv_i8_post_ok(const mhip_conv_i8_t *p);
+size_t mhip_conv_i8_post_pack(int c, const int8_t *packed, const int32_t *bias, int8_t *out);
+int mhip_conv_i8_post_k(int c, int k);
+int mhip_conv_i8_post_row(int c, int oc);
 int mhip_conv_i8_oc_row(int oc, int oc_pad);
 int mhip_conv_i8_pre_ok(const mhip_conv_i8_t *p);
 size_t mhip_conv_i8_rgb_pack(int in_c, int kh, int kw, int stride_h, int stride_w, int pad_left, int oc_pad, int k64,
```
